# lich0031/AIDE

Hardware: AMD Instinct MI355X
Metric: training images/sec FuseUNet 256x256x2 bs=4/GPU (higher is better)
Workload: dtype f32; 1 GPU; c2 fuseunet fwd+loss+bwd+Adam(amsgrad), 256x256 2-modal, bs=4/GPU, fp32; global_batch=4, parallelism=dp1

## Files before the change

aide_amd/build.py:

```python
import hashlib
import os
import subprocess
import sys
from concurrent.futures import ThreadPoolExecutor

HERE = os.path.dirname(os.path.abspath(__file__))
CSRC = os.path.join(HERE, 'csrc')
OBJ = os.path.join(HERE, 'build')
LIB = os.path.join(HERE, 'libaide_hip.so')
SOURCES = ['conv3x3.hip', 'conv3x3_winograd.hip', 'conv3x3_wino4.hip', 'conv3x3_wgrad.hip', 'conv3x3_wgrad4.hip', 'conv3x3_wgrad_stem.hip', 'conv3x3_bf16.hip', 'bn.hip', 'spatial.hip', 'loss.hip', 'loss_mc.hip', 'coteach_ext.hip', 'head_adam.hip',
           'convt.hip', 'attention.hip', 'ktimer.hip', 'eval3d.hip', 'augment.hip', 'labelbank.hip', 'labelbank_image.hip', 'metrics_mc.hip']
FLAGS = ['--offload-arch=gfx950', '-O3', '-std=c++17', '-fPIC', '-ffp-contract=fast']


def _hipcc():
    for c in (os.environ.get('HIPCC'), '/opt/rocm/bin/hipcc', 'hipcc'):
        if c and (os.path.isabs(c) and os.path.exists(c) or not os.path.isabs(c)):
            return c
    raise RuntimeError('hipcc not found')


def _digest(paths):
    h = hashlib.sha1()
    for p in paths:
        with open(p, 'rb') as f:
            h.update(f.read())
    h.update(' '.join(FLAGS).encode())
    return h.hexdigest()


def build(force=False, verbose=True):
    os.makedirs(OBJ, exist_ok=True)
    hipcc = _hipcc()
    common = os.path.join(CSRC, 'common.h')

    def compile_one(src):
        sp = os.path.join(CSRC, src)
        op = os.path.join(OBJ, src.replace('.hip', '.o'))
        stamp = op + '.sha1'
        dg = _digest([sp, common])
        if not force and os.path.exists(op) and os.path.exists(stamp) and open(stamp).read() == dg:
            return op, False
        cmd = [hipcc] + FLAGS + ['-c', sp, '-o', op]
        r = subprocess.run(cmd, capture_output=True, text=True)
        if r.returncode != 0:
            raise RuntimeError('hipcc failed for %s:\n%s' % (src, r.stderr))
        with open(stamp, 'w') as f:
            f.write(dg)
        return op, True

    with ThreadPoolExecutor(max_workers=4) as ex:
        results = list(ex.map(compile_one, SOURCES))
    objs = [o for o, _ in results]
    if force or any(ch for _, ch in results) or not os.path.exists(LIB):
        r = subprocess.run([hipcc, '--offload-arch=gfx950', '-shared', '-fPIC', '-o', LIB] + objs,
                           capture_output=True, text=True)
        if r.returncode != 0:
            raise RuntimeError('link failed:\n' + r.stderr)
        if verbose:
            print('built', LIB)
    elif verbose:
        print('up to date', LIB)
    return LIB


if __name__ == '__main__':
    build(force='--force' in sys.argv)
```

aide_amd/csrc/conv3x3_wino4.hip:

```cpp
#include "common.h"
#include <stdlib.h>
#include <type_traits>

namespace {

template <int V> using ic = std::integral_constant<int, V>;

struct W4Args {
    const float* x;
    const float* u;
    const float* bias;
    float* y;
    long x_bs, y_bs, split_stride;
    int N, Cin, H, W, Cout;
    int blocks_w, blocks_h, n_co_tiles, splitk, stages_total, accumulate;
    int gp, gc;
    int pair;
    float* stats;
    const float* scale;
    int relu;
    const float* in_tab;
    int in_ng;
};

constexpr int F4_BNIN_MAXC = 1024;
constexpr int F4_NAGPR = 16;
constexpr int F4_RRS = 41;
constexpr int F4_RCS = 775;
constexpr int F4_RAW = 4 * F4_RCS;
constexpr int F4_V = 36 * 32 * 4;
constexpr int F4_SET = F4_RAW + F4_V;
constexpr int F4_LDS = 2 * F4_SET > 4 * 128 * 64 ? 2 * F4_SET : 4 * 128 * 64;

__host__ __device__ constexpr int f4_pos(int q, int b) {
    return 6 * (q / 3) + ((q % 3) == 0 ? 1 + b : (q % 3) == 1 ? 3 + b : 5 * b);
}
__host__ __device__ constexpr int f4_slot(int c) { return c == 0 ? 4 : c == 5 ? 5 : c - 1; }

__device__ __forceinline__ void bt6(float d0, float d1, float d2, float d3, float d4, float d5, float* o, int st) {
    const float a = __builtin_fmaf(-4.f, d2, d4), b = __builtin_fmaf(4.f, d1, -d3);
    const float c = d4 - d2, e = d3 - d1;
    o[0] = __builtin_fmaf(-5.f, d2, __builtin_fmaf(4.f, d0, d4));
    o[st] = a - b;
    o[2 * st] = a + b;
    o[3 * st] = __builtin_fmaf(2.f, e, c);
    o[4 * st] = __builtin_fmaf(-2.f, e, c);
    o[5 * st] = __builtin_fmaf(-5.f, d3, __builtin_fmaf(4.f, d1, d5));
}

template <int CTRL, int ROW_MASK>
__device__ __forceinline__ float dpp_add(float v) {
    return v + __builtin_bit_cast(float, __builtin_amdgcn_update_dpp(0, __builtin_bit_cast(int, v), CTRL, ROW_MASK, 0xf, true));
}
__device__ __forceinline__ float half_total_dpp(float v) {
    v = dpp_add<0x111, 0xf>(v);
    v = dpp_add<0x112, 0xf>(v);
    v = dpp_add<0x114, 0xf>(v);
    v = dpp_add<0x118, 0xf>(v);
    v = dpp_add<0x142, 0xa>(v);
    return v;
}

template <int MODE, bool AFF = false, bool BNIN = false>
__global__ __launch_bounds__(256, 1) void conv3x3_wino4_kernel(const W4Args a) {
    extern __shared__ __attribute__((aligned(16))) float lds[];
    const int tid = threadIdx.x, lane = tid & 63;
    const int wid = __builtin_amdgcn_readfirstlane(tid >> 6);
    const int half = lane >> 5, j = lane & 31;
    const int ph = wid & 1, cb = wid >> 1;

    int b = xcd_remap(blockIdx.x, gridDim.x);
    const int p_in = b % a.gp;            b /= a.gp;
    const int co_in = b % a.gc;           b /= a.gc;
    const int ncg = a.n_co_tiles / a.gc;
    const int cog = b % ncg;              b /= ncg;
    const int split = b % a.splitk;       b /= a.splitk;
    const int co_tile = cog * a.gc + co_in;
    int pt = b * a.gp + p_in;
    const int tw = pt % a.blocks_w;       pt /= a.blocks_w;
    const int th = pt % a.blocks_h;
    const int n = pt / a.blocks_h;
    constexpr int PAIR = MODE == 1;
    constexpr bool canv = MODE == 2;
    constexpr int NR = canv ? 22 : 18, NI = canv ? 5 : 8, RRS = canv ? 29 : F4_RRS;
    constexpr int TPH = canv ? 20 : 16, TPW = canv ? 20 : 32;
    static_assert(NR * RRS <= F4_RCS, "raw channel plane");
    const int h0 = th * TPH, w0 = tw * TPW, co0 = co_tile * 64;
    const int HW = a.H * a.W;
    constexpr int pair = PAIR;

    const int sps = a.stages_total / a.splitk;
    const int s_begin = split * sps;
    const int s_end = min(s_begin + sps, a.stages_total);

    constexpr int NUI = 4 * NR * NI, NUE = 4 * NR * 2;
    unsigned offB[3], ldsB[3], offC, ldsC;
    int tabB[3], tabC;
#pragma unroll
    for (int e = 0; e < 3; ++e) {
        int q = tid + e * 256;
        while (q >= NUI) q -= 256;
        const int c = q / (NR * NI), rem = q - c * (NR * NI), r = rem / NI, s4 = rem - r * NI;
        const int ih = h0 - 1 + r, iw = w0 + 4 * s4;
        const int imgB = pair && s4 >= 4;
        const bool ok = ih >= 0 && ih < a.H && (pair || iw < a.W);
        offB[e] = ok ? (unsigned)((long)imgB * a.x_bs + c * HW + r * a.W + 1 + 4 * (pair ? (s4 & 3) : s4)) * 4u : BUF_OOB;
        ldsB[e] = (unsigned)(c * F4_RCS + r * RRS + 4 + 4 * s4 + 2 * imgB);
        tabB[e] = F4_LDS + (ok ? 0 : 2 * a.Cin) + 2 * c;
    }
    {
        int q = tid;
        if (q >= NUE) q -= NUE;
        const int c = q / (NR * 2), rem = q - c * (NR * 2), r = rem >> 1, side = rem & 1;
        const int ih = h0 - 1 + r, iw = side ? w0 + TPW : w0 - 1;
        const bool ok = !pair && ih >= 0 && ih < a.H && iw >= 0 && iw < a.W;
        tabC = F4_LDS + (ok ? 0 : 2 * a.Cin) + 2 * c;
        offC = ok ? (unsigned)(c * HW + r * a.W + (side ? TPW + 1 : 0)) * 4u : BUF_OOB;
        ldsC = (unsigned)(c * F4_RCS + r * RRS + (pair ? (side ? 21 : 20) : (side ? 4 + TPW : 3)));
    }
    const __amdgpu_buffer_rsrc_t xrs =
        make_rsrc(a.x + (long)(pair ? 2 * n : n) * a.x_bs + (long)h0 * a.W + w0 - (a.W + 1));
    const long ubase = ((long)9 * ph * 2 * a.Cout + co0 + cb * 32) * 4;
    const __amdgpu_buffer_rsrc_t urs = __builtin_amdgcn_make_buffer_rsrc(
        const_cast<float*>(a.u + ubase), 0, (int)(((long)a.Cin * 36 * a.Cout - ubase) * 4), 0x00020000);
    const unsigned uoff = (unsigned)(half * a.Cout + j) * 16u;
    const unsigned upos = (unsigned)a.Cout * 32u;

    f32x4 rb[3];
    float rc;
    f32x4 ua[2][9];
    auto fetch_u = [&](int q, int stage, f32x4* dst) {
        const unsigned us = ((unsigned)min(stage, s_end - 1) * 18u + (unsigned)q) * upos;
        dst[q] = buf_load_f32x4(urs, uoff, us);
    };
    auto fetch = [&](int l, int stage) {
        const unsigned xs = (unsigned)(min(stage, s_end - 1) * 4) * (unsigned)HW * 4u;
        if (l < 3) rb[l] = buf_load_f32x4(xrs, offB[l], xs);
        else rc = buf_load_f32(xrs, offC, xs);
    };
    auto put_raw = [&](int w, float* raw) {
        if (w < 12) raw[ldsB[w >> 2] + (w & 3)] = rb[w >> 2][w & 3];
        else raw[ldsC] = rc;
    };
    f32x2 tv[4];
    auto bn_tab = [&](int stage) {
        const int so = min(stage, s_end - 1) * 8;
#pragma unroll
        for (int e = 0; e < 3; ++e) tv[e] = *reinterpret_cast<const f32x2*>(lds + tabB[e] + so);
        tv[3] = *reinterpret_cast<const f32x2*>(lds + tabC + so);
    };
    auto bn_in = [&]() {
#pragma unroll
        for (int e = 0; e < 3; ++e) {
            const f32x2 sc = f32x2{tv[e].x, tv[e].x}, sh = f32x2{tv[e].y, tv[e].y};
            const f32x2 lo = f32x2{rb[e].x, rb[e].y} * sc + sh, hi = f32x2{rb[e].z, rb[e].w} * sc + sh;
            rb[e] = f32x4{fmaxf(lo.x, 0.f), fmaxf(lo.y, 0.f), fmaxf(hi.x, 0.f), fmaxf(hi.y, 0.f)};
        }
        rc = fmaxf(__builtin_fmaf(rc, tv[3].x, tv[3].y), 0.f);
    };
    if constexpr (BNIN) {
        float* tab = lds + F4_LDS;
        const float* src = a.in_tab + (long)(n / a.in_ng) * 2 * a.Cin;
        for (int i = tid; i < 2 * a.Cin; i += 256) { tab[i] = src[i]; tab[2 * a.Cin + i] = 0.f; }
        __syncthreads();
    }

    const int item = tid & 127, hs = wid >> 1;
    const int tslot = canv ? min(item >> 2, 24) : (item >> 2);
    const int trow = canv ? tslot / 5 : tslot >> 3, tcol = canv ? tslot - 5 * trow : tslot & 7;
    const int xr_off = (item & 3) * F4_RCS + trow * 4 * RRS + 3 + 4 * tcol + ((pair && tcol >= 4) ? 2 : 0);
    f32x2 tp[6][3];
    f32x2 tq[9];
    auto xf_read = [&](int i, int xo) {
        const float v = lds[xo + (i / 6) * RRS + (i % 6)];
        if ((i % 6) & 1) tp[i / 6][(i % 6) >> 1].y = v; else tp[i / 6][(i % 6) >> 1].x = v;
    };
    auto xf_half = [&](auto HS) {
        constexpr int khs = decltype(HS)::value;
        f32x2 T[3][3];
#pragma unroll
        for (int cp = 0; cp < 3; ++cp) {
            const f32x2 d0 = tp[0][cp], d1 = tp[1][cp], d2 = tp[2][cp], d3 = tp[3][cp], d4 = tp[4][cp], d5 = tp[5][cp];
            if (khs == 0) {
                const f32x2 aa = d4 - 4.f * d2, bb = 4.f * d1 - d3;
                T[0][cp] = (4.f * d0 + d4) - 5.f * d2;
                T[1][cp] = bb * f32x2{-1.f, -1.f} + aa;
                T[2][cp] = aa + bb;
            } else {
                const f32x2 cc = d2 * f32x2{-1.f, -1.f} + d4, ee = d1 * f32x2{-1.f, -1.f} + d3;
// ... 78 lines not shown
            if constexpr (BNIN) {
                if (st == 24) bn_tab(s + 2);
                if (st == 30) bn_in();
            }
            if (st >= PR && st < PR + 5) {
#pragma unroll
                for (int q = 0; q < 3; ++q)
                    if (3 * (st - PR) + q < 13) put_raw(3 * (st - PR) + q, sc);
            }
            __builtin_amdgcn_sched_barrier(0);
        }
        __syncthreads();
    };
    for (int s = s_begin; s < s_end; s += 2) {
        stage(s, set0, set1, ic<0>{});
        stage(s + 1, set1, set0, ic<1>{});
    }

    float* xbuf = lds;
    float* yn = a.y + (long)split * a.split_stride + (long)(pair ? 2 * n + ((j & 7) >> 2) : n) * a.y_bs;
    const bool add_bias = (a.bias != nullptr) && (split == 0);
    const int oh = h0 + 4 * (canv ? j / 5 : j >> 3), ow = pair ? 4 * (j & 3) : w0 + 4 * (canv ? j % 5 : j & 7);
    const bool pok = (!canv || j < 25) && oh < a.H && ow < a.W;
    auto epilogue = [&](auto PH) {
        constexpr int kph = decltype(PH)::value;
        auto partial = [&](int r, f32x2* yp) {
            f32x2 T[3][4];
#pragma unroll
            for (int i = 0; i < 3; ++i) {
                auto m = [&](int c) { return f32x2{acc[6 * i + f4_slot(c)][r], acc[6 * i + f4_slot(c)][r + 1]}; };
                const f32x2 m0 = m(0), m1 = m(1), m2 = m(2), m3 = m(3), m4 = m(4), m5 = m(5);
                const f32x2 s12 = m1 + m2, d12 = m2 * f32x2{-1.f, -1.f} + m1, s34 = m3 + m4, d34 = m4 * f32x2{-1.f, -1.f} + m3;
                T[i][0] = m0 + s12 + s34;
                T[i][1] = d34 * f32x2{2.f, 2.f} + d12;
                T[i][2] = s34 * f32x2{4.f, 4.f} + s12;
                T[i][3] = d34 * f32x2{8.f, 8.f} + d12 + m5;
            }
#pragma unroll
            for (int bq = 0; bq < 4; ++bq) {
                if (kph == 0) {
                    const f32x2 sm = T[1][bq] + T[2][bq], df = T[2][bq] * f32x2{-1.f, -1.f} + T[1][bq];
                    yp[bq] = T[0][bq] + sm; yp[4 + bq] = df; yp[8 + bq] = sm; yp[12 + bq] = df;
                } else {
                    const f32x2 sm = T[0][bq] + T[1][bq], df = T[1][bq] * f32x2{-1.f, -1.f} + T[0][bq];
                    yp[bq] = sm; yp[4 + bq] = df * f32x2{2.f, 2.f}; yp[8 + bq] = sm * f32x2{4.f, 4.f};
                    yp[12 + bq] = df * f32x2{8.f, 8.f} + T[2][bq];
                }
            }
        };
        f32x2* const xbuf2 = reinterpret_cast<f32x2*>(xbuf);
#pragma unroll
        for (int rp = 0; rp < 4; ++rp) {
            f32x2 yp[16];
            partial(2 * rp + 8 * (1 - kph), yp);
#pragma unroll
            for (int o = 0; o < 16; ++o) xbuf2[((wid * 64) + rp * 16 + o) * 64 + lane] = yp[o];
        }
        __syncthreads();
        float bvs[8];
#pragma unroll
        for (int q = 0; q < 8; ++q) {
            const int r = q + 8 * kph;
            const int co = co0 + cb * 32 + (r & 3) + 8 * (r >> 2) + 4 * half;
            bvs[q] = (add_bias && co < a.Cout) ? a.bias[co] : 0.f;
        }
        float svs[8];
        if constexpr (AFF) {
#pragma unroll
            for (int q = 0; q < 8; ++q) {
                const int r = q + 8 * kph;
                const int co = co0 + cb * 32 + (r & 3) + 8 * (r >> 2) + 4 * half;
                svs[q] = co < a.Cout ? a.scale[co] : 1.f;
            }
        }
#pragma unroll
        for (int rp = 0; rp < 4; ++rp) {
            f32x2 yp[16];
            partial(2 * rp + 8 * kph, yp);
#pragma unroll
            for (int o = 0; o < 16; ++o) yp[o] += xbuf2[(((wid ^ 1) * 64) + rp * 16 + o) * 64 + lane];
#pragma unroll
            for (int e = 0; e < 2; ++e) {
                const int r = 2 * rp + e + 8 * kph;
                const int co = co0 + cb * 32 + (r & 3) + 8 * (r >> 2) + 4 * half;
                if (a.stats) {
                    float s1 = 0.f, s2 = 0.f;
                    if (pok) {
#pragma unroll
                        for (int o = 0; o < 16; ++o) { s1 += yp[o][e]; s2 = __builtin_fmaf(yp[o][e], yp[o][e], s2); }
                    }
                    s1 = half_total_dpp(s1);
                    s2 = half_total_dpp(s2);
                    if (j == 31 && co < a.Cout) {
                        const int nparts = a.N * a.blocks_h * a.blocks_w, blk = (n * a.blocks_h + th) * a.blocks_w + tw;
                        *reinterpret_cast<f32x2*>(a.stats + ((long)co * nparts + blk) * 2) = f32x2{s1, s2};
                    }
                }
                if (pok && co < a.Cout) {
                    const float bv = bvs[2 * rp + e];
                    f32x4* const p0 = reinterpret_cast<f32x4*>(yn + (long)co * HW + (long)oh * a.W + ow);
                    f32x4 o[4];
#pragma unroll
                    for (int i = 0; i < 4; ++i)
                        o[i] = f32x4{yp[4 * i][e] + bv, yp[4 * i + 1][e] + bv, yp[4 * i + 2][e] + bv, yp[4 * i + 3][e] + bv};
                    if constexpr (AFF) {
                        const float sv = svs[2 * rp + e];
#pragma unroll
                        for (int i = 0; i < 4; ++i) {
#pragma unroll
                            for (int k = 0; k < 4; ++k) {
                                const float v = __builtin_fmaf(yp[4 * i + k][e], sv, bv);
                                o[i][k] = a.relu ? fmaxf(v, 0.f) : v;
                            }
                        }
                    }
                    if (a.accumulate) {
                        f32x4 old[4];
#pragma unroll
                        for (int i = 0; i < 4; ++i) old[i] = *reinterpret_cast<const f32x4*>(reinterpret_cast<const float*>(p0) + (long)i * a.W);
#pragma unroll
                        for (int i = 0; i < 4; ++i) o[i] += old[i];
                    }
#pragma unroll
                    for (int i = 0; i < 4; ++i) *reinterpret_cast<f32x4*>(reinterpret_cast<float*>(p0) + (long)i * a.W) = o[i];
                }
            }
        }
    };
    if (ph == 0) epilogue(ic<0>{}); else epilogue(ic<1>{});
    };
    if (hs == 0) run(ic<0>{}); else run(ic<1>{});
}

__global__ __launch_bounds__(256) void w4_splitk_reduce_kernel(const float* __restrict__ slabs, long split_stride,
                                                               int splitk, float* __restrict__ y, long y_bs, int C,
                                                               int HW, const float* __restrict__ bias, int accumulate,
                                                               long total4, const float* __restrict__ scale, int relu) {
    for (long i = (long)blockIdx.x * 256 + threadIdx.x; i < total4; i += (long)gridDim.x * 256) {
        const long e = i * 4, chw = (long)C * HW;
        const long n = e / chw, rem = e - n * chw;
        f32x4 v = *reinterpret_cast<const f32x4*>(slabs + e);
        for (int s = 1; s < splitk; ++s) v += *reinterpret_cast<const f32x4*>(slabs + (long)s * split_stride + e);
        if (scale) {
            const float sv = scale[rem / HW], bv = bias[rem / HW];
#pragma unroll
            for (int k = 0; k < 4; ++k) { const float t = __builtin_fmaf(v[k], sv, bv); v[k] = relu ? fmaxf(t, 0.f) : t; }
        } else if (bias) { const float bv = bias[rem / HW]; v += f32x4{bv, bv, bv, bv}; }
        f32x4* p = reinterpret_cast<f32x4*>(y + n * y_bs + rem);
        if (accumulate) v += *p;
        *p = v;
    }
}

__device__ __forceinline__ void wino4_g(const float g[9], float u[36]) {
    float t[18];
#pragma unroll
    for (int c = 0; c < 3; ++c) {
        const float g0 = g[c], g1 = g[3 + c], g2 = g[6 + c];
        const float s = g0 + g2;
        t[c] = 0.25f * g0;
        t[3 + c] = (-1.f / 6.f) * (s + g1);
        t[6 + c] = (-1.f / 6.f) * (s - g1);
        const float q = __builtin_fmaf(4.f, g2, g0);
        t[9 + c] = (1.f / 24.f) * (q + 2.f * g1);
        t[12 + c] = (1.f / 24.f) * (q - 2.f * g1);
        t[15 + c] = g2;
    }
#pragma unroll
    for (int r = 0; r < 6; ++r) {
        const float a0 = t[r * 3], a1 = t[r * 3 + 1], a2 = t[r * 3 + 2];
        const float s = a0 + a2, q = __builtin_fmaf(4.f, a2, a0);
        u[r * 6] = 0.25f * a0;
        u[r * 6 + 1] = (-1.f / 6.f) * (s + a1);
        u[r * 6 + 2] = (-1.f / 6.f) * (s - a1);
        u[r * 6 + 3] = (1.f / 24.f) * (q + 2.f * a1);
        u[r * 6 + 4] = (1.f / 24.f) * (q - 2.f * a1);
        u[r * 6 + 5] = a2;
    }
}

struct W4PackDesc {
    const float* w; float* uf; float* ud;
    int Co, Ci, pad0, pad1;
    long block_start;
};

constexpr int P4_T = 32;
__global__ __launch_bounds__(128) void wino4_pack_multi_kernel(const W4PackDesc* __restrict__ descs, int n, long total_blocks) {
    __shared__ __attribute__((aligned(16))) float ot[36 * 128];
    for (long blk = blockIdx.x; blk < total_blocks; blk += gridDim.x) {
    int lo = 0, hi = n - 1;
    while (lo < hi) {
        const int mid = (lo + hi + 1) >> 1;
        if (descs[mid].block_start <= blk) lo = mid; else hi = mid - 1;
    }
    const W4PackDesc d = descs[lo];
    const int tid = threadIdx.x;
    const int tiles_ci = (d.Ci + P4_T - 1) / P4_T;
    const int tb = (int)(blk - d.block_start);
    const int co0 = (tb / tiles_ci) * P4_T, ci0 = (tb % tiles_ci) * P4_T;
    const int nci = min(P4_T, d.Ci - ci0);
    float g[9], u[36];
    const int lo2 = tid & 3, hi5 = tid >> 2;
    for (int grp = 0; grp < 16; ++grp) {
        const bool fwd = grp < 8;
        const int q = grp & 7;
        float* dst = fwd ? d.uf : d.ud;
        if (dst == nullptr) continue;
        const int co = fwd ? hi5 : 4 * q + lo2, ci = fwd ? 4 * q + lo2 : hi5;
        const bool live = fwd ? (ci0 + 4 * q < d.Ci) : (co0 + 4 * q < d.Co);
        if (!live) continue;
        {
            const bool in = co0 + co < d.Co && ci < nci;
            const float* wp = d.w + ((long)(co0 + co) * d.Ci + ci0 + ci) * 9;
#pragma unroll
            for (int t = 0; t < 9; ++t) g[t] = in ? wp[fwd ? t : 8 - t] : 0.f;
        }
        wino4_g(g, u);
        const int otid = (lo2 >> 1) * 64 + hi5 * 2 + (lo2 & 1);
#pragma unroll
        for (int p = 0; p < 36; ++p) ot[p * 128 + otid] = u[p];
        __syncthreads();
        const int C = fwd ? d.Co : d.Ci, c0 = fwd ? co0 : ci0;
        const long gbase = (long)((fwd ? ci0 : co0) / 4 + q) * 18;
        const int nrow = min(P4_T, C - c0);
#pragma unroll
        for (int k = 0; k < 9; ++k) {
            const int f = tid + k * 128, pq = f >> 6, hh = (f >> 5) & 1, row = f & 31;
            if (row < nrow) {
                const float* o0 = ot + f4_pos(pq, 0) * 128 + hh * 64 + row * 2;
                const float* o1 = ot + f4_pos(pq, 1) * 128 + hh * 64 + row * 2;
                *reinterpret_cast<f32x4*>(dst + (((gbase + pq) * 2 + hh) * C + c0 + row) * 4) =
                    f32x4{o0[0], o0[1], o1[0], o1[1]};
            }
        }
        __syncthreads();
    }
    }
}

}

extern "C" {

int aide_conv3x3_wino4_supported(int Cin, int H, int W, int Cout) {
    return (H % 4 == 0 && W % 4 == 0 && H >= 16 && W >= 16 && Cout % 32 == 0 &&
            Cin % 8 == 0) ? 1 : 0;
}

static int f4_mode(int H, int W, int* bh, int* bw) {
    const int sh = (H + 15) / 16, sw = (W + 31) / 32, ch = (H + 19) / 20, cw = (W + 19) / 20;
    const int mode = W == 16 ? 1 : ((long)ch * cw < (long)sh * sw) ? 2 : 0;
    *bh = mode == 2 ? ch : sh;
    *bw = mode == 2 ? cw : sw;
    return mode;
}

int aide_conv3x3_wino4_splitk(int N, int Cin, int H, int W, int Cout) {
    int bh, bw;
    f4_mode(H, W, &bh, &bw);
    const long nb = (long)bh * bw * (W == 16 ? N / 2 : N) * ((Cout + 63) / 64);
    const int pairs = Cin / 8;
    const long target = 200;
    int s = 1;
    while (nb * s < target && pairs % (s * 2) == 0 && s * 2 <= pairs / 4) s *= 2;
    return s;
}

int aide_conv3x3_wino4_stats_parts(int N, int H, int W) {
    int bh, bw;
    f4_mode(H, W, &bh, &bw);
    return W < 32 ? 0 : N * bh * bw;
}

int aide_conv3x3_wino4_pack_blocks(int Co, int Ci) {
    return ((Co + P4_T - 1) / P4_T) * ((Ci + P4_T - 1) / P4_T);
}

int aide_conv3x3_wino4_pack_multi(const void* descs, int n, int64_t total_blocks, hipStream_t stream) {
    if (!descs || n <= 0 || total_blocks <= 0) return AIDE_ERR_ARG;
    static_assert(sizeof(W4PackDesc) == 48, "descriptor layout");
    const long grid = total_blocks;
    AIDE_LAUNCH_TIMED(AIDE_KT_OTHER, 0.0, wino4_pack_multi_kernel, dim3((unsigned)grid), dim3(128), 0, stream,
                       (const W4PackDesc*)descs, n, (long)total_blocks);
    return aide_launch_status();
}

int aide_conv3x3_wino4(const float* x, int64_t x_bs, const float* u, const float* bias, float* y,
                       int64_t y_bs, int N, int Cin, int H, int W, int Cout, int accumulate, int splitk,
                       float* ws, float* stats_parts, const float* epi_scale, int epi_relu, const float* in_bn_tab,
                       int in_bn_group_images, hipStream_t stream) {
    const float* aff = epi_scale;
    const int aff_relu = aff ? epi_relu : 0;
    if (!x || !u || !y || !aide_conv3x3_wino4_supported(Cin, H, W, Cout) || x_bs % 4 || y_bs % 4 || (W == 16 && N % 2))
        return AIDE_ERR_ARG;
    static AideLdsOptIn lds_opt;
    if (int rc = lds_opt.ensure([] {
            constexpr int plain = F4_LDS * (int)sizeof(float), bnin = (F4_LDS + 4 * F4_BNIN_MAXC) * (int)sizeof(float);
            const struct { const void* fn; int bytes; } ks[] = {
                {(const void*)conv3x3_wino4_kernel<0>, plain}, {(const void*)conv3x3_wino4_kernel<1>, plain},
                {(const void*)conv3x3_wino4_kernel<2>, plain}, {(const void*)conv3x3_wino4_kernel<0, true>, plain},
                {(const void*)conv3x3_wino4_kernel<2, true>, plain}, {(const void*)conv3x3_wino4_kernel<0, false, true>, bnin},
                {(const void*)conv3x3_wino4_kernel<2, false, true>, bnin}};
            for (const auto& k : ks) {
                const hipError_t e = hipFuncSetAttribute(k.fn, hipFuncAttributeMaxDynamicSharedMemorySize, k.bytes);
                if (e != hipSuccess) return e;
            }
            return hipSuccess;
        })) return rc;
    W4Args a;
    if (stats_parts && !(splitk <= 1 && accumulate == 0 && W >= 32)) return AIDE_ERR_ARG;
    a.stats = stats_parts;
    const int mode = f4_mode(H, W, &a.blocks_h, &a.blocks_w);
    if (aff && (accumulate != 0 || !bias || (mode == 1 && splitk <= 1))) return AIDE_ERR_ARG;
    a.scale = splitk > 1 ? nullptr : aff;
    a.relu = aff_relu;
    a.pair = mode == 1 ? 1 : 0;
    if (in_bn_tab && (mode == 1 || aff || Cin > F4_BNIN_MAXC || in_bn_group_images < 1 || N % in_bn_group_images)) return AIDE_ERR_ARG;
    a.in_tab = in_bn_tab; a.in_ng = in_bn_tab ? in_bn_group_images : 1;
    a.x = x; a.u = u; a.x_bs = x_bs; a.N = N; a.Cin = Cin; a.H = H; a.W = W; a.Cout = Cout;
    a.n_co_tiles = (Cout + 63) / 64;
    a.stages_total = Cin / 4;
    if (splitk < 1) splitk = 1;
    if ((Cin / 8) % splitk != 0) return AIDE_ERR_ARG;
    if (splitk > 1 && !ws) return AIDE_ERR_ARG;
    a.splitk = splitk;
    if (splitk > 1) {
        a.y = ws; a.y_bs = (long)Cout * H * W; a.split_stride = (long)N * Cout * H * W;
        a.bias = nullptr; a.accumulate = 0;
    } else {
        a.y = y; a.y_bs = y_bs; a.split_stride = 0; a.bias = bias; a.accumulate = (accumulate == 1);
    }
    const long nb = (long)a.blocks_w * a.blocks_h * (a.pair ? N / 2 : N) * a.n_co_tiles * splitk;
    {
        const long P = (long)a.blocks_w * a.blocks_h * (a.pair ? N / 2 : N);
        const int C = a.n_co_tiles;
        const long per_xcd = nb / 8 > 0 ? nb / 8 : 1;
        const double ub = 144.0 * (double)Cin * Cout, xb = 1.44 * 4.0 * (double)N * Cin * H * W;
        long bp = 1; int bc = C;
        double best = 1e300;
        const bool grouped = AIDE_CONV_FLOPS(N, H, W, Cout, Cin) >= 8e9;
        for (long gp = 1; gp <= P && gp <= per_xcd && grouped; gp *= 2) {
            if (P % gp) continue;
            for (int gc = 1; gc <= C; ++gc) {
                if (C % gc || gp * gc > per_xcd) continue;
                const double cost = ub * (double)P / (double)gp + xb * (double)C / (double)gc;
                if (cost < best) { best = cost; bp = gp; bc = gc; }
            }
        }
        a.gp = (int)bp; a.gc = bc;
    }
    if (a.in_tab) {
        const size_t lds_bytes = (F4_LDS + 4 * (size_t)Cin) * sizeof(float);
        if (mode == 2) {
            AIDE_LAUNCH_TIMED(AIDE_KT_WINO4, AIDE_CONV_FLOPS(N, H, W, Cout, Cin), (conv3x3_wino4_kernel<2, false, true>),
                              dim3((unsigned)nb), dim3(256), lds_bytes, stream, a);
        } else {
            AIDE_LAUNCH_TIMED(AIDE_KT_WINO4, AIDE_CONV_FLOPS(N, H, W, Cout, Cin), (conv3x3_wino4_kernel<0, false, true>),
                              dim3((unsigned)nb), dim3(256), lds_bytes, stream, a);
        }
    } else if (a.scale && mode == 2) {
        AIDE_LAUNCH_TIMED(AIDE_KT_WINO4, AIDE_CONV_FLOPS(N, H, W, Cout, Cin), (conv3x3_wino4_kernel<2, true>), dim3((unsigned)nb),
                          dim3(256), F4_LDS * sizeof(float), stream, a);
    } else if (a.scale) {
        AIDE_LAUNCH_TIMED(AIDE_KT_WINO4, AIDE_CONV_FLOPS(N, H, W, Cout, Cin), (conv3x3_wino4_kernel<0, true>), dim3((unsigned)nb),
                          dim3(256), F4_LDS * sizeof(float), stream, a);
    } else if (a.pair) {
        AIDE_LAUNCH_TIMED(AIDE_KT_WINO4, AIDE_CONV_FLOPS(N, H, W, Cout, Cin), conv3x3_wino4_kernel<1>, dim3((unsigned)nb), dim3(256),
                          F4_LDS * sizeof(float), stream, a);
    } else if (mode == 2) {
        AIDE_LAUNCH_TIMED(AIDE_KT_WINO4, AIDE_CONV_FLOPS(N, H, W, Cout, Cin), conv3x3_wino4_kernel<2>, dim3((unsigned)nb), dim3(256),
                          F4_LDS * sizeof(float), stream, a);
    } else {
        AIDE_LAUNCH_TIMED(AIDE_KT_WINO4, AIDE_CONV_FLOPS(N, H, W, Cout, Cin), conv3x3_wino4_kernel<0>, dim3((unsigned)nb), dim3(256),
                          F4_LDS * sizeof(float), stream, a);
    }
    int rc = aide_launch_status();
    if (rc != 0) return rc;
    if (splitk > 1 && accumulate != 2) {
        const long total4 = (long)N * Cout * H * W / 4;
        AIDE_LAUNCH_TIMED(AIDE_KT_REDUCE, 0.0, w4_splitk_reduce_kernel, dim3((unsigned)min((total4 + 255) / 256, 4096L)), dim3(256), 0,
                           stream, ws, (long)N * Cout * H * W, splitk, y, (long)y_bs, Cout, H * W, bias, accumulate,
                           total4, aff, aff_relu);
        rc = aide_launch_status();
    }
    return rc;
}

}
```

aide_amd/csrc/conv3x3_winograd.hip:

```cpp
#include "common.h"

namespace {

struct WinoArgs {
    const float* x;
    const float* u;
    const float* bias;
    float* y;
    long x_bs, y_bs, split_stride;
    int N, Cin, H, W, Cout;
    int tiles_w, tiles_h, n_co_tiles, splitk, chunks_total, accumulate;
};

constexpr int WCK = 8;
constexpr int WTCO = 64;
constexpr int RROWS = 18, RRS = 24;
constexpr int RCS = RROWS * RRS + 8;
constexpr int RAWL = WCK * RCS;
constexpr int VL = 16 * 64 * WCK;
constexpr int UL = 16 * WTCO * WCK;
constexpr int WBUF = RAWL + VL + UL;

__global__ __launch_bounds__(256, 1) void conv3x3_wino_kernel(const WinoArgs a) {
    extern __shared__ __attribute__((aligned(16))) float lds[];
    const int tid = threadIdx.x, lane = tid & 63, wid = tid >> 6;
    const int half = lane >> 5, j = lane & 31;
    const int wave_m = wid >> 1, wave_n = wid & 1;

    int b = xcd_remap(blockIdx.x, gridDim.x);
    const int co_tile = b % a.n_co_tiles; b /= a.n_co_tiles;
    const int split = b % a.splitk;       b /= a.splitk;
    const int tw = b % a.tiles_w;         b /= a.tiles_w;
    const int th = b % a.tiles_h;
    const int n = b / a.tiles_h;
    const int h0 = th * 16, w0 = tw * 16, co0 = co_tile * WTCO;
    const int HW = a.H * a.W;

    const int cps = (a.chunks_total + a.splitk - 1) / a.splitk;
    const int c_begin = split * cps;
    const int c_end = min(c_begin + cps, a.chunks_total);

    constexpr int NRB = 3, NRC = 2, NU = UL / 4 / 256;
    unsigned offB[NRB], ldsB[NRB], offC[NRC], ldsC[NRC], offU[NU];
#pragma unroll
    for (int e = 0; e < NRB; ++e) {
        int q = tid + e * 256;
        if (q >= WCK * RROWS * 4) q -= 256;
        const int c = q / (RROWS * 4), rem = q - c * (RROWS * 4), r = rem / 4, s4 = rem - r * 4;
        const int ih = h0 - 1 + r, iw = w0 + 4 * s4;
        const bool ok = ih >= 0 && ih < a.H && iw < a.W;
        offB[e] = ok ? (unsigned)(c * HW + r * a.W + 1 + 4 * s4) * 4u : BUF_OOB;
        ldsB[e] = (unsigned)(c * RCS + r * RRS + 4 + 4 * s4);
    }
#pragma unroll
    for (int e = 0; e < NRC; ++e) {
        int q = tid + e * 256;
        if (q >= WCK * RROWS * 2) q -= 256;
        const int c = q / (RROWS * 2), rem = q - c * (RROWS * 2), r = rem / 2, side = rem - r * 2;
        const int ih = h0 - 1 + r, iw = side ? w0 + 16 : w0 - 1;
        const bool ok = ih >= 0 && ih < a.H && iw >= 0 && iw < a.W;
        offC[e] = ok ? (unsigned)(c * HW + r * a.W + (side ? 17 : 0)) * 4u : BUF_OOB;
        ldsC[e] = (unsigned)(c * RCS + r * RRS + (side ? 20 : 3));
    }
#pragma unroll
    for (int v = 0; v < NU; ++v) {
        const int f = tid + v * 256;
        const int pp = f / (WTCO * WCK / 4), w4 = f - pp * (WTCO * WCK / 4);
        offU[v] = (unsigned)(pp * a.Cout * WCK + w4 * 4) * 4u;
    }
    const __amdgpu_buffer_rsrc_t xrs =
        make_rsrc(a.x + (long)n * a.x_bs + (long)h0 * a.W + w0 - (a.W + 1));
    const __amdgpu_buffer_rsrc_t urs = make_rsrc(a.u + (long)co0 * WCK);

    f32x4 rb[NRB], ru[NU];
    float rc[NRC];
    auto fetch_raw = [&](int l, int chunk) {
        const unsigned xs = (unsigned)(min(chunk, c_end - 1) * WCK) * (unsigned)HW * 4u;
        if (l < NRB) rb[l] = buf_load_f32x4(xrs, offB[l], xs);
        else rc[l - NRB] = buf_load_f32(xrs, offC[l - NRB], xs);
    };
    auto put_raw = [&](int l, float* raw) {
        if (l < NRB) *reinterpret_cast<f32x4*>(raw + ldsB[l]) = rb[l];
        else raw[ldsC[l - NRB]] = rc[l - NRB];
    };
    auto fetch_u = [&](int v, int chunk) {
        const unsigned us = (unsigned)min(chunk, c_end - 1) * 16u * (unsigned)a.Cout * (unsigned)WCK * 4u;
        ru[v] = buf_load_f32x4(urs, offU[v], us);
    };
    auto put_u = [&](int v, float* ubuf) { *reinterpret_cast<f32x4*>(ubuf + (tid + v * 256) * 4) = ru[v]; };

    f32x2 td[16], to[16];
    const int xci = lane & 7, xtj = lane >> 3;
    const int xr_off = xci * RCS + 4 * wid * RRS + 3 + 2 * xtj;
    const int xw_off = (2 * wid * 8 + xtj) * WCK + xci;
    auto xf_read = [&](int i, const float* raw) {
        td[i].x = raw[xr_off + (i / 4) * RRS + (i % 4)];
        td[i].y = raw[xr_off + (2 + i / 4) * RRS + (i % 4)];
    };
    auto xf_math = [&]() {
        f32x2 tt[16];
#pragma unroll
        for (int c = 0; c < 4; ++c) {
            tt[c] = td[c] - td[8 + c]; tt[4 + c] = td[4 + c] + td[8 + c];
            tt[8 + c] = td[8 + c] - td[4 + c]; tt[12 + c] = td[4 + c] - td[12 + c];
        }
#pragma unroll
        for (int r = 0; r < 4; ++r) {
            to[r * 4] = tt[r * 4] - tt[r * 4 + 2]; to[r * 4 + 1] = tt[r * 4 + 1] + tt[r * 4 + 2];
            to[r * 4 + 2] = tt[r * 4 + 2] - tt[r * 4 + 1]; to[r * 4 + 3] = tt[r * 4 + 1] - tt[r * 4 + 3];
        }
    };
    auto xf_store = [&](int o, float* vbuf) {
        vbuf[o * 64 * WCK + xw_off] = to[o].x;
        vbuf[o * 64 * WCK + xw_off + 8 * WCK] = to[o].y;
    };

    f32x16 acc[16];
#pragma unroll
    for (int p = 0; p < 16; ++p)
#pragma unroll
        for (int r = 0; r < 16; ++r) acc[p][r] = 0.0f;

    float* set0 = lds;
    float* set1 = lds + WBUF;
#pragma unroll
    for (int l = 0; l < NRB + NRC; ++l) fetch_raw(l, c_begin);
#pragma unroll
    for (int v = 0; v < NU; ++v) fetch_u(v, c_begin);
#pragma unroll
    for (int l = 0; l < NRB + NRC; ++l) put_raw(l, set0);
#pragma unroll
    for (int v = 0; v < NU; ++v) put_u(v, set0 + RAWL + VL);
#pragma unroll
    for (int l = 0; l < NRB + NRC; ++l) fetch_raw(l, c_begin + 1);
    __syncthreads();
#pragma unroll
    for (int i = 0; i < 16; ++i) xf_read(i, set0);
    xf_math();
#pragma unroll
    for (int o = 0; o < 16; ++o) xf_store(o, set0 + RAWL);
#pragma unroll
    for (int l = 0; l < NRB + NRC; ++l) put_raw(l, set1);
    __syncthreads();

    int cur = 0;
    for (int chunk = c_begin; chunk < c_end; ++chunk) {
        float* sc = cur ? set1 : set0;
        float* sn = cur ? set0 : set1;
        const float* la = sc + RAWL + VL + (wave_m * 32 + j) * WCK + half * 4;
        const float* lb = sc + RAWL + (wave_n * 32 + j) * WCK + half * 4;
        constexpr int STEPS = 16 * (WCK / 2);
        f32x4 a0A, b0A, a1A, b1A, a0B, b0B, a1B, b1B;
        auto frag = [&](int p, f32x4& af, f32x4& bf) {
            af = *reinterpret_cast<const f32x4*>(la + p * WTCO * WCK);
            bf = *reinterpret_cast<const f32x4*>(lb + p * 64 * WCK);
        };
        auto slot = [&](int st, const f32x4& a0c, const f32x4& b0c, const f32x4& a1c, const f32x4& b1c,
                        f32x4& a0n, f32x4& b0n, f32x4& a1n, f32x4& b1n) {
            const int g2 = st >> 3, k = st & 7, q = k >> 1;
            if (k == 0 && g2 + 1 < 8) { frag(2 * g2 + 2, a0n, b0n); frag(2 * g2 + 3, a1n, b1n); }
            if (k & 1) acc[2 * g2 + 1] = __builtin_amdgcn_mfma_f32_32x32x2f32(a1c[q], b1c[q], acc[2 * g2 + 1], 0, 0, 0);
            else acc[2 * g2] = __builtin_amdgcn_mfma_f32_32x32x2f32(a0c[q], b0c[q], acc[2 * g2], 0, 0, 0);
            if (st < NU) fetch_u(st, chunk + 1);
            else if (st < NU + NRB + NRC) fetch_raw(st - NU, chunk + 2);
            if (st >= 4 && st < 20) xf_read(st - 4, sn);
            if (st == 24) xf_math();
            if (st >= 26 && st < 42) xf_store(st - 26, sn + RAWL);
            if (st >= 44 && st < 44 + NU) put_u(st - 44, sn + RAWL + VL);
            if (st >= 52 && st < 52 + NRB + NRC) put_raw(st - 52, sc);
            __builtin_amdgcn_sched_barrier(0);
        };
        frag(0, a0A, b0A); frag(1, a1A, b1A);
#pragma unroll
        for (int st = 0; st < STEPS; st += 16) {
#pragma unroll
            for (int k = 0; k < 8; ++k) slot(st + k, a0A, b0A, a1A, b1A, a0B, b0B, a1B, b1B);
#pragma unroll
            for (int k = 0; k < 8; ++k) slot(st + 8 + k, a0B, b0B, a1B, b1B, a0A, b0A, a1A, b1A);
        }
        __syncthreads();
        cur ^= 1;
    }

    float* yn = a.y + (long)split * a.split_stride + (long)n * a.y_bs;
    const bool add_bias = (a.bias != nullptr) && (split == 0);
    const int tile = wave_n * 32 + j, ti = tile >> 3, tj = tile & 7;
    const int oh = h0 + 2 * ti, ow = w0 + 2 * tj;
    const bool pok = oh < a.H && ow < a.W;
    float bvs[16];
#pragma unroll
    for (int r = 0; r < 16; ++r) {
        const int co = co0 + wave_m * 32 + (r & 3) + 8 * (r >> 2) + 4 * half;
        bvs[r] = (add_bias && pok && co < a.Cout) ? a.bias[co] : 0.f;
    }
#pragma unroll
    for (int r4 = 0; r4 < 16; r4 += 4) {
        float2 olds[4][2];
#pragma unroll
        for (int q = 0; q < 4; ++q) {
            const int co = co0 + wave_m * 32 + q + 8 * (r4 >> 2) + 4 * half;
#pragma unroll
            for (int i = 0; i < 2; ++i)
                olds[q][i] = (a.accumulate && pok && co < a.Cout)
                                 ? *reinterpret_cast<const float2*>(yn + (long)co * HW + (long)(oh + i) * a.W + ow) : make_float2(0.f, 0.f);
        }
#pragma unroll
        for (int q = 0; q < 4; ++q) {
            const int r = r4 + q;
            const int co = co0 + wave_m * 32 + (r & 3) + 8 * (r >> 2) + 4 * half;
            float s[2][4];
#pragma unroll
            for (int c = 0; c < 4; ++c) {
                const float m0 = acc[c][r], m1 = acc[4 + c][r], m2 = acc[8 + c][r], m3 = acc[12 + c][r];
                s[0][c] = m0 + m1 + m2;
                s[1][c] = m1 - m2 - m3;
            }
            if (pok && co < a.Cout) {
                const float bv = bvs[r];
#pragma unroll
                for (int i = 0; i < 2; ++i) {
                    float2 o;
                    o.x = s[i][0] + s[i][1] + s[i][2] + bv;
                    o.y = s[i][1] - s[i][2] - s[i][3] + bv;
                    float2* p = reinterpret_cast<float2*>(yn + (long)co * HW + (long)(oh + i) * a.W + ow);
                    o.x += olds[q][i].x; o.y += olds[q][i].y;
                    *p = o;
                }
            }
        }
    }
}

__global__ void wino_splitk_reduce_kernel(const float* __restrict__ slabs, long split_stride, int splitk,
                                          float* __restrict__ y, long y_bs, int C, int HW,
                                          const float* __restrict__ bias, int accumulate, long total) {
    for (long i = (long)blockIdx.x * blockDim.x + threadIdx.x; i < total;
         i += (long)gridDim.x * blockDim.x) {
        const long chw = (long)C * HW;
        const long n = i / chw, rem = i - n * chw;
        float v = slabs[i];
        for (int s = 1; s < splitk; ++s) v += slabs[(long)s * split_stride + i];
        if (bias) v += bias[rem / HW];
        float* p = y + n * y_bs + rem;
        if (accumulate) v += *p;
        *p = v;
    }
}
__global__ __launch_bounds__(256) void wino_splitk_reduce4_kernel(const float* __restrict__ slabs, long split_stride, int splitk,
                                                                  float* __restrict__ y, long y_bs, int C, int HW,
                                                                  const float* __restrict__ bias, int accumulate, long total4) {
    const long i = (long)blockIdx.x * blockDim.x + threadIdx.x;
    if (i >= total4) return;
    const long chw4 = (long)C * HW / 4;
    const long n = i / chw4, rem = (i - n * chw4) * 4;
    const float* sp = slabs + i * 4;
    f32x4 v = *reinterpret_cast<const f32x4*>(sp);
    int s = 1;
    for (; s + 4 <= splitk; s += 4) {
        const f32x4 t0 = *reinterpret_cast<const f32x4*>(sp + (long)s * split_stride);
        const f32x4 t1 = *reinterpret_cast<const f32x4*>(sp + (long)(s + 1) * split_stride);
        const f32x4 t2 = *reinterpret_cast<const f32x4*>(sp + (long)(s + 2) * split_stride);
        const f32x4 t3 = *reinterpret_cast<const f32x4*>(sp + (long)(s + 3) * split_stride);
        v = (((v + t0) + t1) + t2) + t3;
    }
    for (; s < splitk; ++s) v += *reinterpret_cast<const f32x4*>(sp + (long)s * split_stride);
    if (bias) v += bias[rem / HW];
    float* p = y + n * y_bs + rem;
    if (accumulate) v += *reinterpret_cast<const f32x4*>(p);
    *reinterpret_cast<f32x4*>(p) = v;
}

struct WinoPackDesc {
    const float* w; float* uf; float* ud;
    int Co, Ci, ci_pad, co_pad;
    long block_start;
};

__device__ __forceinline__ void wino_g(const float g[9], float u[16]) {
    float t[12];
#pragma unroll
    for (int c = 0; c < 3; ++c) {
        const float g0 = g[c], g1 = g[3 + c], g2 = g[6 + c];
        t[c] = g0; t[3 + c] = 0.5f * (g0 + g1 + g2); t[6 + c] = 0.5f * (g0 - g1 + g2); t[9 + c] = g2;
    }
#pragma unroll
    for (int r = 0; r < 4; ++r) {
        const float a0 = t[r * 3], a1 = t[r * 3 + 1], a2 = t[r * 3 + 2];
        u[r * 4] = a0; u[r * 4 + 1] = 0.5f * (a0 + a1 + a2); u[r * 4 + 2] = 0.5f * (a0 - a1 + a2); u[r * 4 + 3] = a2;
    }
}

constexpr int WP_T = 32;
__global__ __launch_bounds__(256) void wino_pack_multi_kernel(const WinoPackDesc* __restrict__ descs, int n) {
    __shared__ __attribute__((aligned(16))) float ot[16 * 256];
    const long blk = blockIdx.x;
    int lo = 0, hi = n - 1;
    while (lo < hi) {
        const int mid = (lo + hi + 1) >> 1;
        if (descs[mid].block_start <= blk) lo = mid; else hi = mid - 1;
    }
    const WinoPackDesc d = descs[lo];
    const int tid = threadIdx.x;
    const int tiles_ci = (d.Ci + WP_T - 1) / WP_T;
    const int tb = (int)(blk - d.block_start);
    const int co0 = (tb / tiles_ci) * WP_T, ci0 = (tb % tiles_ci) * WP_T;
    const int nci = min(WP_T, d.Ci - ci0);
    float g[9], u[16];
    const int lo3 = tid & 7, hi5 = tid >> 3;
    for (int grp = 0; grp < 8; ++grp) {
        const bool fwd = grp < 4;
        const int q = grp & 3;
        float* dst = fwd ? d.uf : d.ud;
        if (dst == nullptr) continue;
        const int co = fwd ? hi5 : 8 * q + lo3, ci = fwd ? 8 * q + lo3 : hi5;
        const bool live = fwd ? (ci0 + 8 * q < d.ci_pad) : (co0 + 8 * q < d.co_pad);
        if (!live) continue;
        {
            const bool in = co0 + co < d.Co && ci < nci;
            const float* wp = d.w + ((long)(co0 + co) * d.Ci + ci0 + ci) * 9;
#pragma unroll
            for (int t = 0; t < 9; ++t) g[t] = in ? wp[fwd ? t : 8 - t] : 0.f;
        }
        wino_g(g, u);
#pragma unroll
        for (int p = 0; p < 16; ++p) ot[p * 256 + tid] = u[p];
        __syncthreads();
        const int C = fwd ? d.Co : d.Ci, c0 = fwd ? co0 : ci0;
        const long gbase = (long)((fwd ? ci0 : co0) / 8 + q) * 16;
        const int nrun = min(WP_T, C - c0) * 8;
#pragma unroll
        for (int k = 0; k < 4; ++k) {
            const int f = tid + k * 256, p = f >> 6, x4 = (f & 63) * 4;
            if (x4 < nrun)
                *reinterpret_cast<f32x4*>(dst + ((gbase + p) * C + c0) * 8 + x4) =
                    *reinterpret_cast<const f32x4*>(ot + p * 256 + x4);
        }
        __syncthreads();
    }
}

}

extern "C" {

int aide_conv3x3_wino_supported(int Cin, int H, int W, int Cout) {
    return (H % 2 == 0 && W % 4 == 0 && Cout % 64 == 0 && Cin % 8 == 0) ? 1 : 0;
}

int aide_conv3x3_wino_splitk(int N, int Cin, int H, int W, int Cout) {
    const long nb = (long)((H + 15) / 16) * ((W + 15) / 16) * N * (Cout / 64);
    const int chunks = Cin / 8;
    int s = 1;
    while (nb * s < 200 && s * 2 <= chunks / 4) s *= 2;
    return s;
}

int aide_conv3x3_wino_pack_blocks(int Co, int Ci) {
    return ((Co + WP_T - 1) / WP_T) * ((Ci + WP_T - 1) / WP_T);
}

int aide_conv3x3_wino_pack_multi(const void* descs, int n, int64_t total_blocks, hipStream_t stream) {
    if (!descs || n <= 0 || total_blocks <= 0) return AIDE_ERR_ARG;
    static_assert(sizeof(WinoPackDesc) == 48, "descriptor layout");
    AIDE_LAUNCH_TIMED(AIDE_KT_OTHER, 0.0, wino_pack_multi_kernel, dim3((unsigned)total_blocks), dim3(256), 0, stream,
                       (const WinoPackDesc*)descs, n);
    return aide_launch_status();
}

int aide_conv3x3_wino(const float* x, int64_t x_bs, const float* u, const float* bias, float* y,
                      int64_t y_bs, int N, int Cin, int H, int W, int Cout, int accumulate, int splitk,
                      float* ws, hipStream_t stream) {
    if (!x || !u || !y || !aide_conv3x3_wino_supported(Cin, H, W, Cout) || x_bs % 4 || y_bs % 2)
        return AIDE_ERR_ARG;
    static AideLdsOptIn lds_opt;
    if (int rc = lds_opt.ensure([] {
            return hipFuncSetAttribute((const void*)conv3x3_wino_kernel, hipFuncAttributeMaxDynamicSharedMemorySize,
                                       2 * WBUF * (int)sizeof(float));
        })) return rc;
    WinoArgs a;
    a.x = x; a.u = u; a.x_bs = x_bs; a.N = N; a.Cin = Cin; a.H = H; a.W = W; a.Cout = Cout;
    a.tiles_w = (W + 15) / 16; a.tiles_h = (H + 15) / 16; a.n_co_tiles = Cout / WTCO;
    a.chunks_total = Cin / WCK;
    if (splitk < 1) splitk = 1;
    if (splitk > a.chunks_total) splitk = a.chunks_total;
    if (splitk > 1 && !ws) return AIDE_ERR_ARG;
    a.splitk = splitk;
    if (splitk > 1) {
        a.y = ws; a.y_bs = (long)Cout * H * W; a.split_stride = (long)N * Cout * H * W;
        a.bias = nullptr; a.accumulate = 0;
    } else {
        a.y = y; a.y_bs = y_bs; a.split_stride = 0; a.bias = bias; a.accumulate = (accumulate == 1);
    }
    const long nb = (long)a.tiles_w * a.tiles_h * N * a.n_co_tiles * splitk;
    AIDE_LAUNCH_TIMED(AIDE_KT_WINO2, AIDE_CONV_FLOPS(N, H, W, Cout, Cin), conv3x3_wino_kernel, dim3((unsigned)nb), dim3(256),
                      2 * WBUF * sizeof(float), stream, a);
    int rc = aide_launch_status();
    if (rc != 0) return rc;
    if (splitk > 1 && accumulate != 2) {
        const long total = (long)N * Cout * H * W;
        if ((H * W) % 4 == 0 && y_bs % 4 == 0) {
            AIDE_LAUNCH_TIMED(AIDE_KT_REDUCE, 0.0, wino_splitk_reduce4_kernel, dim3((unsigned)((total / 4 + 255) / 256)), dim3(256), 0, stream, ws,
                               total, splitk, y, (long)y_bs, Cout, H * W, bias, accumulate, total / 4);
        } else {
            const int blocks = (int)min((total + 255) / 256, (long)2048);
            AIDE_LAUNCH_TIMED(AIDE_KT_REDUCE, 0.0, wino_splitk_reduce_kernel, dim3(blocks), dim3(256), 0, stream, ws,
                               total, splitk, y, (long)y_bs, Cout, H * W, bias, accumulate, total);
        }
        rc = aide_launch_status();
    }
    return rc;
}

}
```

aide_amd/csrc/head_adam.hip:

```cpp
#include "common.h"

namespace {

constexpr int MAXK = 8;
constexpr int HEAD_WG_BLOCKS = 1024;

template <int K, typename XT>
__global__ __launch_bounds__(256) void head_fwd_kernel(const XT* __restrict__ x, long x_bs,
                                                       const float* __restrict__ w, const float* __restrict__ b,
                                                       float* __restrict__ y, long y_bs, int C, int HW,
                                                       long total4, const float* __restrict__ in_scale,
                                                       const float* __restrict__ in_shift) {
    extern __shared__ float ws[];
    for (int i = threadIdx.x; i < K * C; i += 256) ws[i] = w[i];
    __syncthreads();
    const int hw4 = HW / 4;
    for (long i = (long)blockIdx.x * 256 + threadIdx.x; i < total4; i += (long)gridDim.x * 256) {
        const long n = i / hw4, p = i - n * hw4;
        const XT* xp = x + n * x_bs + p * 4;
        f32x4 acc[K];
#pragma unroll
        for (int k = 0; k < K; ++k) { const float bk = b ? b[k] : 0.f; acc[k] = f32x4{bk, bk, bk, bk}; }
        for (int c = 0; c < C; ++c) {
            f32x4 v = ld4(xp + (long)c * HW);
            if (in_scale) {
                const float sc = in_scale[c], sh = in_shift[c];
#pragma unroll
                for (int e = 0; e < 4; ++e) v[e] = fmaxf(__builtin_fmaf(v[e], sc, sh), 0.0f);
            }
#pragma unroll
            for (int k = 0; k < K; ++k) acc[k] += ws[k * C + c] * v;
        }
#pragma unroll
        for (int k = 0; k < K; ++k) *reinterpret_cast<f32x4*>(y + n * y_bs + (long)k * HW + p * 4) = acc[k];
    }
}

template <int K, typename DT>
__global__ __launch_bounds__(256) void head_dgrad_kernel(const float* __restrict__ dy, long dy_bs,
                                                         const float* __restrict__ w, DT* __restrict__ dx,
                                                         long dx_bs, int C, int HW, long total4) {
    extern __shared__ float ws[];
    for (int i = threadIdx.x; i < K * C; i += 256) ws[i] = w[i];
    __syncthreads();
    const int hw4 = HW / 4;
    for (long i = (long)blockIdx.x * 256 + threadIdx.x; i < total4; i += (long)gridDim.x * 256) {
        const long n = i / hw4, p = i - n * hw4;
        f32x4 g[K];
#pragma unroll
        for (int k = 0; k < K; ++k) g[k] = *reinterpret_cast<const f32x4*>(dy + n * dy_bs + (long)k * HW + p * 4);
        DT* xp = dx + n * dx_bs + p * 4;
        for (int c = 0; c < C; ++c) {
            f32x4 v = ws[c] * g[0];
#pragma unroll
            for (int k = 1; k < K; ++k) {
                const float wk = ws[k * C + c];
                v = f32x4{__builtin_fmaf(wk, g[k][0], v[0]), __builtin_fmaf(wk, g[k][1], v[1]), __builtin_fmaf(wk, g[k][2], v[2]),
                          __builtin_fmaf(wk, g[k][3], v[3])};
            }
            st4(xp + (long)c * HW, v);
        }
    }
}

template <int K, typename XT>
__global__ __launch_bounds__(256) void head_wgrad_kernel(const float* __restrict__ dy, long dy_bs,
                                                         const XT* __restrict__ x, long x_bs, int C, int HW,
                                                         long total4, double* __restrict__ partials,
                                                         const float* __restrict__ in_scale, const float* __restrict__ in_shift) {
    constexpr int G = K > 4 ? 4 : 8;
    __shared__ double sm[4][G * K];
    const int hw4 = HW / 4;
    const int lane = threadIdx.x & 63, wid = threadIdx.x >> 6;
    const int stride = gridDim.x * 256;
    for (int c0 = -1; c0 < C; c0 += G) {
        double acc[G][K];
#pragma unroll
        for (int g = 0; g < G; ++g)
#pragma unroll
            for (int k = 0; k < K; ++k) acc[g][k] = 0.0;
        for (long i = (long)blockIdx.x * 256 + threadIdx.x; i < total4; i += stride) {
            const long n = i / hw4, p = i - n * hw4;
            f32x4 gk[K];
#pragma unroll
            for (int k = 0; k < K; ++k) gk[k] = *reinterpret_cast<const f32x4*>(dy + n * dy_bs + (long)k * HW + p * 4);
            f32x4 v[G];
#pragma unroll
            for (int g = 0; g < G; ++g) {
                const int c = c0 + g;
                v[g] = f32x4{1.f, 1.f, 1.f, 1.f};
                if (c >= 0 && c < C) {
                    v[g] = ld4(x + n * x_bs + (long)c * HW + p * 4);
                    if (in_scale) {
                        const float sc = in_scale[c], sh = in_shift[c];
#pragma unroll
                        for (int e = 0; e < 4; ++e) v[g][e] = fmaxf(__builtin_fmaf(v[g][e], sc, sh), 0.0f);
                    }
                }
            }
#pragma unroll
            for (int g = 0; g < G; ++g)
#pragma unroll
                for (int k = 0; k < K; ++k)
                    acc[g][k] += (double)(gk[k][0] * v[g][0] + gk[k][1] * v[g][1] + (gk[k][2] * v[g][2] + gk[k][3] * v[g][3]));
        }
#pragma unroll
        for (int g = 0; g < G; ++g)
#pragma unroll
            for (int k = 0; k < K; ++k) acc[g][k] = wave_sum_d(acc[g][k]);
        __syncthreads();
        if (lane == 0)
#pragma unroll
            for (int g = 0; g < G; ++g)
#pragma unroll
                for (int k = 0; k < K; ++k) sm[wid][g * K + k] = acc[g][k];
        __syncthreads();
        if (threadIdx.x < G * K) {
            const int g = threadIdx.x / K, k = threadIdx.x - g * K, c = c0 + g;
            if (c < C) {
                const double t = sm[0][threadIdx.x] + sm[1][threadIdx.x] + sm[2][threadIdx.x] + sm[3][threadIdx.x];
                const int slot = (c >= 0) ? k * C + c : K * C + k;
                partials[(long)blockIdx.x * (K * C + K) + slot] = t;
            }
        }
    }
}

__global__ __launch_bounds__(64) void head_wgrad_finalize_kernel(const double* __restrict__ partials, int nblocks,
                                                                 int KC, int K, float* __restrict__ dw,
                                                                 float* __restrict__ db) {
    const int i = blockIdx.x;
    double s = 0.0;
    for (int b = threadIdx.x; b < nblocks; b += 64) s += partials[(long)b * (KC + K) + i];
    s = wave_sum_d(s);
    if (threadIdx.x == 0) {
        if (i < KC) dw[i] = (float)s;
        else if (db) db[i - KC] = (float)s;
    }
}

struct AdamArgs {
    float* const* p; const float* const* g; float* const* m; float* const* v; float* const* vmax;
    const long* sizes; const long* block_start;
    int ntensors;
    float lr, beta1, beta2, eps, weight_decay, bc1, bc2_sqrt;
    int amsgrad;
};

__global__ __launch_bounds__(256) void adam_kernel(const AdamArgs a) {
    const long blk = blockIdx.x;
    int lo = 0, hi = a.ntensors - 1;
    while (lo < hi) {
        const int mid = (lo + hi + 1) >> 1;
        if (a.block_start[mid] <= blk) lo = mid; else hi = mid - 1;
    }
    const int t = lo;
    const long base = (blk - a.block_start[t]) * 1024;
    const long n = a.sizes[t];
    float* p = a.p[t]; const float* g = a.g[t];
    float* m = a.m[t]; float* v = a.v[t]; float* vm = a.vmax[t];
#pragma unroll
    for (int k = 0; k < 4; ++k) {
        const long i = base + k * 256 + threadIdx.x;
        if (i < n) {
            float gi = g[i];
            const float pi = p[i];
            if (a.weight_decay != 0.f) gi += a.weight_decay * pi;
            const float mi = a.beta1 * m[i] + (1.f - a.beta1) * gi;
            const float vi = a.beta2 * v[i] + (1.f - a.beta2) * gi * gi;
            m[i] = mi; v[i] = vi;
            float vhat = vi;
            if (a.amsgrad) { vhat = fmaxf(vm[i], vi); vm[i] = vhat; }
            const float denom = sqrtf(vhat) / a.bc2_sqrt + a.eps;
            p[i] = pi - (a.lr / a.bc1) * (mi / denom);
        }
    }
}

int grid_for(long total) { return (int)max(1L, min((total + 255) / 256, 4096L)); }

template <int K, typename XT>
int head_wgrad_launch(const float* dy, long dy_bs, const XT* x, long x_bs, int C, int HW, long total4,
                      double* partials, int nblocks, hipStream_t s, const float* in_scale = nullptr, const float* in_shift = nullptr) {
    AIDE_LAUNCH_TIMED(AIDE_KT_OTHER, 0.0, (head_wgrad_kernel<K, XT>), dim3(nblocks), dim3(256), 0, s, dy, dy_bs, x, x_bs, C, HW,
                       total4, partials, in_scale, in_shift);
    return aide_launch_status();
}

template <typename XT>
int head_fwd_t(const XT* x, int64_t x_bs, const float* w, const float* b, float* y, int64_t y_bs, int N, int C, int K,
               int H, int W, hipStream_t stream, const float* in_scale = nullptr, const float* in_shift = nullptr) {
    const int HW = H * W;
    if (K < 1 || K > MAXK || HW % 4 || x_bs % 4 || y_bs % 4) return AIDE_ERR_ARG;
    const long total4 = (long)N * HW / 4;
    const int grid = grid_for(total4);
    const size_t sh = (size_t)K * C * sizeof(float);
    aide_pick<1, 2, 3, 4, 5, 6, 7, 8>(K, [&](auto k) {
        AIDE_LAUNCH_TIMED(AIDE_KT_OTHER, 0.0, (head_fwd_kernel<k(), XT>), dim3(grid), dim3(256), sh, stream, x, (long)x_bs, w, b, y,
                          (long)y_bs, C, HW, total4, in_scale, in_shift);
    });
    return aide_launch_status();
}

template <typename XT, typename DT>
int head_bwd_t(const float* dy, int64_t dy_bs, const XT* x, int64_t x_bs, const float* w, DT* dx, int64_t dx_bs,
               float* dw, float* db, int N, int C, int K, int H, int W, void* ws, hipStream_t stream,
               const float* in_scale = nullptr, const float* in_shift = nullptr) {
    const int HW = H * W;
    if (K < 1 || K > MAXK || HW % 4 || x_bs % 4 || dy_bs % 4 || (dx && dx_bs % 4) || !ws) return AIDE_ERR_ARG;
    const long total4 = (long)N * HW / 4;
    const size_t sh = (size_t)K * C * sizeof(float);
    if (dx) {
        const int grid = grid_for(total4);
        aide_pick<1, 2, 3, 4, 5, 6, 7, 8>(K, [&](auto k) {
            AIDE_LAUNCH_TIMED(AIDE_KT_OTHER, 0.0, (head_dgrad_kernel<k(), DT>), dim3(grid), dim3(256), sh, stream, dy, (long)dy_bs, w, dx,
                              (long)dx_bs, C, HW, total4);
        });
    }
    if (!dw) return aide_launch_status();
    const int nblocks = (int)max(1L, min((total4 + 255) / 256, (long)HEAD_WG_BLOCKS));
    const int rc = aide_pick<1, 2, 3, 4, 5, 6, 7, 8>(K, [&](auto k) {
        return head_wgrad_launch<k()>(dy, dy_bs, x, x_bs, C, HW, total4, (double*)ws, nblocks, stream, in_scale, in_shift);
    });
    if (rc) return rc;
    AIDE_LAUNCH_TIMED(AIDE_KT_OTHER, 0.0, head_wgrad_finalize_kernel, dim3(K * C + K), dim3(64), 0, stream,
                       (const double*)ws, nblocks, K * C, K, dw, db);
    return aide_launch_status();
}

}

extern "C" {

size_t aide_head1x1_ws_bytes(int C, int K) { return (size_t)HEAD_WG_BLOCKS * (K * C + K) * sizeof(double); }

int aide_head1x1_fwd_mixed(const void* x, int x_bf16, int64_t x_bs, const float* w, const float* b, float* y,
                           int64_t y_bs, int N, int C, int K, int H, int W, hipStream_t stream) {
    return aide_with_storage<bf16_store_t>(x_bf16, [&](auto xt) { return head_fwd_t(xt.cast(x), x_bs, w, b, y, y_bs, N, C, K, H, W, stream); });
}
int aide_head1x1_bwd_mixed(const float* dy, int64_t dy_bs, const void* x, int x_bf16, int64_t x_bs, const float* w,
                           void* dx, int dx_bf16, int64_t dx_bs, float* dw, float* db, int N, int C, int K, int H, int W,
                           void* ws, hipStream_t stream) {
    return aide_with_storage<bf16_store_t>(x_bf16, [&](auto xt) { return aide_with_storage<bf16_store_t>(dx_bf16, [&](auto dt) {
        return head_bwd_t(dy, dy_bs, xt.cast(x), x_bs, w, dt.cast(dx), dx_bs, dw, db, N, C, K, H, W, ws, stream);
    }); });
}

int aide_head1x1_fwd_bn(const float* z, int64_t z_bs, const float* in_scale, const float* in_shift, const float* w, const float* b,
                        float* y, int64_t y_bs, int N, int C, int K, int H, int W, hipStream_t stream) {
    if (!z || !in_scale || !in_shift) return AIDE_ERR_ARG;
    return head_fwd_t(z, z_bs, w, b, y, y_bs, N, C, K, H, W, stream, in_scale, in_shift);
}
int aide_head1x1_wgrad_bn(const float* dy, int64_t dy_bs, const float* z, int64_t z_bs, const float* in_scale, const float* in_shift,
                          float* dw, float* db, int N, int C, int K, int H, int W, void* ws, hipStream_t stream) {
    if (!z || !in_scale || !in_shift || !dw) return AIDE_ERR_ARG;
    return head_bwd_t<float, float>(dy, dy_bs, z, z_bs, nullptr, nullptr, 0, dw, db, N, C, K, H, W, ws, stream, in_scale, in_shift);
}

int aide_adam_amsgrad_multi(float* const* p, const float* const* g, float* const* m, float* const* v,
                            float* const* vmax, const int64_t* sizes, const int64_t* block_start,
                            int ntensors, int64_t total_blocks, float lr, float beta1, float beta2, float eps,
                            float weight_decay, int amsgrad, int64_t step, hipStream_t stream) {
    if (ntensors <= 0 || total_blocks <= 0 || step < 1) return AIDE_ERR_ARG;
    AdamArgs a;
    a.p = p; a.g = g; a.m = m; a.v = v; a.vmax = vmax;
    a.sizes = (const long*)sizes; a.block_start = (const long*)block_start; a.ntensors = ntensors;
    a.lr = lr; a.beta1 = beta1; a.beta2 = beta2; a.eps = eps; a.weight_decay = weight_decay;
    a.bc1 = (float)(1.0 - pow((double)beta1, (double)step));
    a.bc2_sqrt = (float)sqrt(1.0 - pow((double)beta2, (double)step));
    a.amsgrad = amsgrad;
    AIDE_LAUNCH_TIMED(AIDE_KT_OTHER, 0.0, adam_kernel, dim3((unsigned)total_blocks), dim3(256), 0, stream, a);
    return aide_launch_status();
}

}
```

aide_amd/engine.py:

```python
import ctypes

import torch

from . import ops
from ._lib import lib, check as _check
from .tape import Tape

PARAM_EPOCH = [0]
STATS_EPOCH = [0]


class GTensor(object):

    def __init__(self, name, channels, level, root=None, c0=0, is_input=False):
        self.name, self.C, self.level = name, channels, level
        self.root = root if root is not None else self
        self.c0 = c0
        self.is_input = is_input

    def slice(self, c0, channels, name=None):
        assert 0 <= c0 and c0 + channels <= self.C
        return GTensor(name or '%s[%d:%d]' % (self.name, c0, c0 + channels), channels, self.level,
                       self.root, self.c0 + c0)


class Graph(object):
    def __init__(self):
        self.roots, self.inputs, self.ops = [], [], []
        self.output = None

    def tensor(self, name, channels, level):
        t = GTensor(name, channels, level)
        self.roots.append(t)
        return t

    def input(self, name, channels):
        t = GTensor(name, channels, 0, is_input=True)
        self.inputs.append(t)
        return t

    def conv_bn_relu(self, src, dst, conv, bn, lane=0):
        self.ops.append(dict(kind='conv', src=src, dst=dst, conv=conv, bn=bn, lane=lane))

    def convT_bn_relu(self, src, dst, conv, bn):
        self.ops.append(dict(kind='convT', src=src, dst=dst, conv=conv, bn=bn))

    def pool(self, src, dst, lane_split=None):
        self.ops.append(dict(kind='pool', src=src, dst=dst, lane_split=lane_split))

    def upsample(self, src, dst):
        self.ops.append(dict(kind='up', src=src, dst=dst))

    def head(self, src, conv):
        self.ops.append(dict(kind='head', src=src, conv=conv))

    def spatial_attention(self, src, dst, mod):
        self.ops.append(dict(kind='sa', src=src, dst=dst, mod=mod))


FAMILIES = ops.FAMILIES
BF16 = ops.BF16
PACK_ORDER = (BF16, 4, 0, 2)
PRECISIONS = ('fp32', 'bf16')
import os as _os


class EngineConfig(object):
    DEFAULTS = dict(
        use_winograd=True,
        use_winograd_dgrad=True,
        use_winograd4=True,
        store_bf16=True,
        store_a_bf16=True,
        store_g_bf16=True,
        replay=_os.environ.get('AIDE_REPLAY', '1') != '0',
        shared_packs=True,
        fold_eval_bn=True,
        tail_wgrad_main=True,
        dual_fwd=True,
        free_lane=True,
        handover_on_kernel=True,
        w4_half_tile=True,
        grouped_bn=True,
        lazy_bn=True,
        direct_grads=_os.environ.get('AIDE_DIRECT_GRADS', '1') != '0',
        fuse_pool_bwd=True,
        fuse_head_bwd=True,
        lazy_head=True,
        fuse_pool_fwd=True,
    )

    def __init__(self, on_change=None):
        object.__setattr__(self, '_on_change', on_change)
        for k, v in self.DEFAULTS.items():
            object.__setattr__(self, k, v)

    def __setattr__(self, k, v):
        if k not in self.DEFAULTS:
            raise AttributeError('aide_amd: the engine has no switch %r (switches: %s)' % (k, ', '.join(sorted(self.DEFAULTS))))
        v = bool(v)
        if getattr(self, k) != v:
            object.__setattr__(self, k, v)
            if self._on_change is not None:
                self._on_change()

    def snapshot(self):
        return tuple(getattr(self, k) for k in sorted(self.DEFAULTS))


FLUSH_EVERY = 4


def conv_mode(cfg, n, cin, h, w, cout):
    if cfg.use_winograd and cfg.use_winograd4 and lib.aide_conv3x3_wino4_supported(cin, h, w, cout) and w != 16:
        flops = 2.0 * n * h * w * cin * cout * 9
        if cout % 64:
            return 0
        if flops >= 8e9 or cin * cout >= 128 * 128:
            return 4
    return 2 if use_winograd(cfg, n, cin, h, w, cout) else 0


WGRAD_OVERRIDE = {}


def use_winograd(cfg, n, cin, h, w, cout):
    return bool(cfg.use_winograd and lib.aide_conv3x3_wino_supported(cin, h, w, cout))


def select_conv(cfg, precision, training, groups, n, cin, cout, h, w, need_dgrad, stem_only_so_far):
    bf16 = precision == 'bf16'
    d = dict(wg_target=0, stats_parts=0)
    d['wino_f'] = conv_mode(cfg, n, cin, h, w, cout)
    d['wino_d'] = conv_mode(cfg, n, cout, h, w, cin) if (need_dgrad and cfg.use_winograd_dgrad) else 0
    if bf16 and FAMILIES[BF16].supported(cin, h, w, cout):
        d['wino_f'] = BF16
    if bf16 and need_dgrad and FAMILIES[BF16].supported(cout, h, w, cin):
        d['wino_d'] = BF16
    d['plan_f'] = FAMILIES[d['wino_f']].plan(n, cin, h, w, cout)
    d['plan_d'] = FAMILIES[d['wino_d']].plan(n, cout, h, w, cin) if need_dgrad else 0
    d['sk_f'] = lib.aide_conv3x3_ws_bytes(n, h, w, cout, d['plan_f'] >> 8)
    d['sk_d'] = lib.aide_conv3x3_ws_bytes(n, h, w, cin, d['plan_d'] >> 8) if need_dgrad else 0
    if bf16 and FAMILIES[BF16].wgrad_supported(cout, cin, h, w):
        d['wino_w'] = BF16
    elif cfg.use_winograd and cfg.use_winograd4 and (cout % 64 == 0 or cfg.w4_half_tile) and \
            WGRAD_OVERRIDE.get((cout, cin, h, w), 4) == 4 and FAMILIES[4].wgrad_supported(cout, cin, h, w):
        d['wino_w'] = 4
        if stem_only_so_far:
            d['wg_target'] = 256
    elif cfg.use_winograd and FAMILIES[2].wgrad_supported(cout, cin, h, w):
        d['wino_w'] = 2
    else:
        d['wino_w'] = 0
    d['wg_bytes'] = FAMILIES[d['wino_w']].wgrad_ws_bytes(n, cout, cin, h, w, **_wgrad_extra(d))
    if training and (d['plan_f'] >> 8) <= 1 \
            and (h * w) % 4 == 0 and lib.aide_bn_two_pass(n // max(groups, 1), cout, h, w):
        parts = lib.aide_conv3x3_wino4_stats_parts(n, h, w) if d['wino_f'] == 4 else 0
        d['stats_parts'] = max(parts, 0)
    d['fold'] = not training and cfg.fold_eval_bn and (
        (d['wino_f'] == 4 and w != 16) or (d['wino_f'] == 0 and (d['plan_f'] >> 8) <= 1))
    d['dz_bf16'] = (d['wino_w'] == BF16 and (not need_dgrad or d['wino_d'] == BF16) and cfg.store_bf16)
    d['z_bf16'] = d['wino_f'] == BF16 and cfg.store_bf16
    return d


def _wgrad_extra(st):
    return dict(target_wgs=256) if st.get('wg_target') else {}


def _pack_slot(mode, direction):
    return ('u' if mode else 'w') + direction


def _preferred(dev):
    from . import streams as _streams
    d = torch.device(dev)
    idx = d.index if d.index is not None else torch.cuda.current_device()
    pref = _streams.PREFERRED.get(idx)
    if pref is None:
        pref = _streams.PREFERRED[idx] = dict(side=torch.cuda.Stream(device=d), lane=torch.cuda.Stream(device=d))
    return pref


def _side_stream(dev):
    return _preferred(dev)['side']


class _Cover(object):

    def __init__(self):
        self.iv = []

    def write(self, c0, c1):
        covered = [(max(a, c0), min(b, c1)) for a, b in self.iv if a < c1 and b > c0]
        if not covered:
            self._add(c0, c1)
            return False, []
        gaps, cur = [], c0
        for a, b in sorted(covered):
            if a > cur:
                gaps.append((cur, a))
            cur = max(cur, b)
        if cur < c1:
            gaps.append((cur, c1))
        self._add(c0, c1)
        return True, gaps

    def _add(self, c0, c1):
        iv = sorted(self.iv + [(c0, c1)])
        out = [iv[0]]
        for a, b in iv[1:]:
            if a <= out[-1][1]:
                out[-1] = (out[-1][0], max(out[-1][1], b))
            else:
                out.append((a, b))
        self.iv = out


class Plan(object):
    def __init__(self, graph, params, n, h, w, device, training, precision='fp32', groups=1, shared=None, cfg=None):
        self.g, self.N, self.H, self.W, self.dev, self.training = graph, n, h, w, device, training
        cfg = self.cfg = cfg if cfg is not None else EngineConfig()
        self.precision = precision
        self._shared = shared if shared is not None else dict(buf={}, fresh={}, streams=None)
        self.groups = groups
        assert n % groups == 0
        bf16 = precision == 'bf16'
        self.pindex = {id(p): i for i, p in enumerate(params)}
        f32 = dict(device=device, dtype=torch.float32)
        forward_only = (groups > 1 or not training) and cfg.shared_packs

        def pack_buf(conv, direction, mode, make):
            key = (id(conv), direction, mode, device.index)
            t = self._shared['buf'].get(key)
            if t is None:
                t = self._shared['buf'][key] = make()
            return t
        self.act = {}
        self.grad = {}
        self.steps = []
        max_dz = max_wg = max_bnc = max_sk = 0
        stem_only = True
        for op in graph.ops:
            st = dict(op)
            if op['kind'] in ('conv', 'convT'):
                conv, src, dst = op['conv'], op['src'], op['dst']
                hh, ww = h >> dst.level, w >> dst.level
                cout = dst.C
                st['z'] = torch.empty(n, cout, hh, ww, **f32)
                for k in ('mean', 'rstd', 'scale', 'shift', 'fbias'):
                    st[k] = torch.empty(cout, **f32)
                max_dz = max(max_dz, n * cout * hh * ww)
                max_bnc = max(max_bnc, cout)
                if op['kind'] == 'conv':
                    cin = src.C
                    need_dg = not src.root.is_input and not forward_only
                    sel = select_conv(cfg, precision, training, groups, n, cin, cout, hh, ww, need_dg, stem_only)
                    max_sk = max(max_sk, sel.pop('sk_f'), sel.pop('sk_d'))
                    st.update(sel)
                    st['wf'] = st['wd'] = st['uf'] = st['ud'] = None
                    for direction, ci, co in [('f', cin, cout)] + ([('d', cout, cin)] if need_dg else []):
                        fam = FAMILIES[st['wino_' + direction]]
                        st[_pack_slot(fam.mode, direction)] = pack_buf(conv, direction, fam.mode,
                                                                       lambda: fam.pack_alloc(ci, co, device))
                    max_wg = max(max_wg, st['wg_bytes'])
                    st['stats'] = torch.empty(cout * st['stats_parts'] * 2, **f32) if st['stats_parts'] else None
                    st['pack_key'] = None
                    st['flops'] = 2.0 * n * hh * ww * cout * cin * 9
                    if st['z_bf16']:
                        st['z'] = torch.empty(n, cout, hh, ww, device=device, dtype=torch.bfloat16)
                else:
                    cin = src.C
                    st['wg_bytes'] = lib.aide_convT2x2_wgrad_ws_bytes(n, cin, cout, h >> src.level, w >> src.level)
                    max_wg = max(max_wg, st['wg_bytes'])
            elif op['kind'] == 'head':
                src = op['src']
                k = op['conv'].out_channels
                max_wg = max(max_wg, lib.aide_head1x1_ws_bytes(src.C, k))
            elif op['kind'] == 'sa':
                src, mod = op['src'], op['mod']
                hh, ww = h >> src.level, w >> src.level
                r = mod.conv1.out_channels
                for k in ('t1', 't2', 't3'):
                    st[k] = torch.empty(n, r, hh, ww, **f32)
                st['t4'] = torch.empty(n, 1, hh, ww, **f32)
                st['gate'] = torch.empty(n, hh, ww, **f32)
                st['stat'] = torch.empty(2, **f32)
            stem_only = stem_only and op['kind'] == 'conv' and op['src'].root.is_input
            self.steps.append(st)
        self._plan_lazy_bn()
        self._plan_lazy_head()
        narrow = {id(t): bf16 and cfg.store_a_bf16 for t in graph.roots}
        for st in self.steps:
            kind = st['kind']
            if kind == 'conv':
                if not (st['wino_f'] == BF16 and st['wino_w'] == BF16):
                    narrow[id(st['src'].root)] = False
            elif kind in ('convT', 'sa'):
                narrow[id(st['src'].root)] = False
            if kind == 'sa':
                narrow[id(st['dst'].root)] = False
        for t in graph.roots:
            dt = torch.bfloat16 if narrow.get(id(t)) else torch.float32
            self.act[id(t)] = torch.empty(n, t.C, h >> t.level, w >> t.level, device=device, dtype=dt)
        self._plan_pool_fwd()
        self.narrow_grad = {k: v and cfg.store_g_bf16 for k, v in narrow.items()}
        for st in self.steps:
            if st['kind'] == 'conv' and not st['src'].root.is_input and st['wino_d'] != BF16:
                self.narrow_grad[id(st['src'].root)] = False
        self.bn_ws = ops.bn_ws(max(max_bnc, 1), device)
        self.sk_ws = torch.empty(max(max_sk // 4, 1), **f32)
        self.lane_b = None
        if any(st.get('lane') for st in self.steps):
            pref = _preferred(device)
            self.lane_b = pref['lane'] if (pref is not None and pref.get('lane') is not None) else torch.cuda.Stream(device=device)
            self.bn_ws_b = ops.bn_ws(max(max_bnc, 1), device)
            self.sk_ws_b = torch.empty(max(max_sk // 4, 1), **f32)
            self.ev_lane_fork, self.ev_lane_join = ops.new_event(), ops.new_event()
            for st in self.steps:
                if st['kind'] == 'pool' and st.get('lane_split'):
                    st['ev_b'] = ops.new_event()
        self._max_dz, self._max_wg = max_dz, max_wg
        self.wg_ws = self.wg_queue = self._wq_active = None
        self._bwd_ready = False
        self.profiler = None
        self._pack_key, self._pack_tabs, self._pack_ids, self.side_fwd = None, {}, None, None
        self.side = _side_stream(device) if (training and groups == 1) else None
        self._convs = self._conv_wslots = None
        self._gate_conv = None
        self._tape_f = self._tape_b = None
        self._coef_key, self._coef_tensors, self._coef_ok, self._coef_next, self._coef_bns = None, None, False, None, []
        self._fp = None
        self._fp_slots = self._fp_bns = None
        self.overlap = True
        self.trace = None
        self.serial = 0
        self.key = None

    def _plan_lazy_bn(self):
        self.lazy_bn = 0
        if not (self.training and self.groups > 1) or not self.cfg.lazy_bn:
            return
        for st in self.steps:
            if st['kind'] != 'conv' or st.get('stats') is None:
                continue
            dst = st['dst']
            readers = [o for o in self.steps if o.get('src') is not None and o['src'].root is dst.root
                       and o['src'].c0 < dst.c0 + dst.C and dst.c0 < o['src'].c0 + o['src'].C]
            if len(readers) != 1:
                continue
            rd = readers[0]
            src = rd['src']
            if rd['kind'] != 'conv' or rd['wino_f'] != 4 or src.C > 1024 or not (src.c0 <= dst.c0 and dst.c0 + dst.C <= src.c0 + src.C):
                continue
            if rd.get('in_tab') is None:
                tab = torch.zeros(self.groups, src.C, 2, device=self.dev, dtype=torch.float32)
                tab[:, :, 0] = 1.0
                rd['in_tab'] = tab
            st['lazy_to'], st['tab_c0'] = rd, dst.c0 - src.c0
            st['z'] = None
            self.lazy_bn += 1

    def _plan_lazy_head(self):
        if not (self.training and self.groups == 1 and self.cfg.lazy_head and self.cfg.fuse_head_bwd):
            return
        for hst in self.steps:
            if hst['kind'] != 'head':
                continue
            src = hst['src']
            readers = [o for o in self.steps if o.get('src') is not None and o['src'].root is src.root
                       and o['src'].c0 < src.c0 + src.C and src.c0 < o['src'].c0 + o['src'].C]
            prods = [o for o in self.steps if o['kind'] == 'conv' and o['dst'].root is src.root
                     and (o['dst'].c0, o['dst'].C) == (src.c0, src.C)]
            if len(readers) != 1 or len(prods) != 1:
                continue
            o = prods[0]
            zn, zc, zh, zw = o['z'].shape
            if o.get('stats') is None or o['z'].dtype != torch.float32 or o.get('dz_bf16') or o.get('lazy_to') is not None or \
                    not lib.aide_bn_one_pass(zn, zc, zh, zw):
                continue
            o['head_lazy'] = True
            o['head_tab'] = torch.zeros(1, zc, 2, device=self.dev, dtype=torch.float32)
            hst['lazy_prod'] = o

    def _plan_pool_fwd(self):
        if not (self.training and self.cfg.fuse_pool_fwd) or (self.groups > 1 and not self.cfg.grouped_bn):
            return
        m = self.N // max(self.groups, 1)
        for pst in self.steps:
            if pst['kind'] != 'pool':
                continue
            src, dst = pst['src'], pst['dst']
            if src.root.is_input or self.act[id(src.root)].dtype != torch.float32 or self.act[id(dst.root)].dtype != torch.float32:
                continue
            prods = [o for o in self.steps if o['kind'] == 'conv' and o['dst'].root is src.root
                     and src.c0 <= o['dst'].c0 and o['dst'].c0 + o['dst'].C <= src.c0 + src.C]
            cover = sorted((o['dst'].c0, o['dst'].c0 + o['dst'].C) for o in prods)
            if not cover or cover[0][0] != src.c0 or cover[-1][1] != src.c0 + src.C or any(a[1] != b[0] for a, b in zip(cover, cover[1:])):
                continue
            ok = True
            for o in prods:
                if o.get('z') is None or o['z'].dtype != torch.float32:
                    ok = False
                    break
                zn, zc, zh, zw = o['z'].shape
                if o.get('stats') is not None or (o['plan_f'] >> 8) > 1 or o.get('lazy_to') is not None or o.get('head_lazy') or \
                        not lib.aide_bn_relu_bwd_pool_supported(m, zc, zh, zw):
                    ok = False
            if not ok:
                continue
            for o in prods:
                o['pool_out'] = dst.slice(o['dst'].c0 - src.c0, o['dst'].C)
            pst['fwd_fused'] = True

    def view(self, t, inputs=None):
        if t.root.is_input:
            x = inputs[self.g.inputs.index(t.root)]
            return x if (t.c0 == 0 and t.C == t.root.C) else x[:, t.c0:t.c0 + t.C]
        buf = self.act[id(t.root)]
        return buf if (t.c0 == 0 and t.C == t.root.C) else buf[:, t.c0:t.c0 + t.C]

    def gview(self, t):
        buf = self.grad[id(t.root)]
        return buf if (t.c0 == 0 and t.C == t.root.C) else buf[:, t.c0:t.c0 + t.C]

    def _prepare_backward(self):
        f32 = dict(device=self.dev, dtype=torch.float32)
        n, h, w = self.N, self.H, self.W
        for t in self.g.roots:
            dt = torch.bfloat16 if self.narrow_grad.get(id(t)) else torch.float32
            self.grad[id(t)] = torch.empty(n, t.C, h >> t.level, w >> t.level, device=self.dev, dtype=dt)
        for st in self.steps:
            if st['kind'] in ('conv', 'convT'):
                st['dz'] = torch.empty(st['z'].shape, device=self.dev,
                                       dtype=torch.bfloat16 if st.get('dz_bf16') else torch.float32)
        off = 0
        for st in self.steps:
            if st['kind'] in ('conv', 'convT'):
                st['wg_off'] = off
                off += (st['wg_bytes'] // 4 + 63) // 64 * 64
        self.wg_ws = torch.empty(max(off, 1), **f32)
        for st in self.steps:
            if st['kind'] in ('conv', 'convT'):
                st['wg_ws'] = self.wg_ws[st['wg_off']:st['wg_off'] + max(st['wg_bytes'] // 4, 1)]
        self.head_ws = torch.empty(max(self._max_wg // 4, 1), **f32)
        self.wg_queue = ops.new_wgrad_queue()
        sa = [st for st in self.steps if st['kind'] == 'sa']
        if sa:
            big = max(st['t1'].numel() for st in sa)
            self.sa_da, self.sa_db = torch.empty(big, **f32), torch.empty(big, **f32)
            self.sa_ws = torch.empty(max(st['gate'].numel() for st in sa) * 2 + 8, **f32)
        if self.side is None:
            self.side = _side_stream(self.dev)
        self.ev_fork, self.ev_join = ops.new_event(), ops.new_event()
        for st in self.steps:
            if st['kind'] in ('conv', 'convT'):
                st['ev'] = ops.new_event()
        cover = {id(t): _Cover() for t in self.g.roots}
        for st in reversed(self.steps):
            src = st['src']
            if src.root.is_input:
                st['src_grad'] = None
                continue
            acc, gaps = cover[id(src.root)].write(src.c0, src.c0 + src.C)
            st['src_grad'] = dict(accumulate=acc, gaps=[src.root.slice(a, b - a) for a, b in gaps])
            if st['kind'] == 'convT' and acc:
                raise NotImplementedError('ConvTranspose input with several consumers')
        for i, st in enumerate(self.steps):
            st['fold_dgrad'] = False
            sg = st.get('src_grad')
            if i == 0 or st['kind'] != 'conv' or sg is None or sg['accumulate'] or sg['gaps']:
                continue
            prod = self.steps[i - 1]
            src, dst = st['src'], prod.get('dst')
            if prod['kind'] != 'conv' or dst is None or dst.root is not src.root or (dst.c0, dst.C) != (src.c0, src.C):
                continue
            if sum(1 for o in self.steps if o.get('src') is not None and o['src'].root is src.root
                   and o['src'].c0 < src.c0 + src.C and src.c0 < o['src'].c0 + o['src'].C) != 1:
                continue
            if st['wino_d'] not in (2, 4) or (st['plan_d'] >> 8) <= 1 or prod.get('dz_bf16') or st.get('dz_bf16'):
                continue
            if self.grad[id(src.root)].dtype != torch.float32 or prod['z'].dtype != torch.float32:
                continue
            pn, pc, ph, pw = prod['z'].shape
            if not lib.aide_bn_one_pass(pn, pc, ph, pw) or (ph * pw) % 4:
                continue
            st['fold_dgrad'] = True
        for st in self.steps:
            st.pop('pool_fuse', None)
# ... 25 lines not shown
                    o['pool_fuse'] = dst.slice(o['dst'].c0 - src.c0, o['dst'].C)
                pst['bwd_fused'] = True
        if self.cfg.fuse_head_bwd:
            for hst in self.steps:
                sg = hst.get('src_grad')
                if hst['kind'] != 'head' or sg is None or sg['accumulate'] or sg['gaps']:
                    continue
                src = hst['src']
                readers = [o for o in self.steps if o.get('src') is not None and o['src'].root is src.root
                           and o['src'].c0 < src.c0 + src.C and src.c0 < o['src'].c0 + o['src'].C]
                prods = [o for o in self.steps if o['kind'] == 'conv' and o['dst'].root is src.root
                         and (o['dst'].c0, o['dst'].C) == (src.c0, src.C)]
                if len(readers) != 1 or len(prods) != 1:
                    continue
                o = prods[0]
                zn, zc, zh, zw = o['z'].shape
                if o['z'].dtype != torch.float32 or o.get('dz_bf16') or o.get('pool_fuse') is not None or \
                        not lib.aide_bn_one_pass(zn, zc, zh, zw) or (zh * zw) % 4:
                    continue
                o['head_fuse'] = hst
                hst['dgrad_fused'] = True
        self._bwd_ready = True

    def _pack_filters(self):
        convs = self._convs
        if convs is None:
            convs = self._convs = [st for st in self.steps if st['kind'] == 'conv']
            self._conv_wslots = [st['conv']._parameters for st in convs]
        ws = [d['weight'] for d in self._conv_wslots]
        key = (PARAM_EPOCH[0],) + tuple((w.data_ptr(), w._version) for w in ws)
        if key == self._pack_key:
            return None
        ptrs = tuple(k[0] for k in key[1:])
        fresh_map = self._shared['fresh']
        mine = self._pack_ids
        if mine is None:
            mine = self._pack_ids = tuple(id(st[k]) for st in convs for k in ('wf', 'wd', 'uf', 'ud') if st[k] is not None)
        fresh = frozenset(i for i in mine if fresh_map.get(i) == key)
        cached = self._pack_tabs.get((ptrs, fresh))
        if cached is None:
            split = min(4, len(convs))

            def tables(group):
                def pick(st, mode, direction):
                    t = st[_pack_slot(mode, direction)] if st['wino_' + direction] == mode else None
                    return None if (t is None or id(t) in fresh) else t
                tabs = {}
                for mode, fam in FAMILIES.items():
                    entries = [(st['conv'].weight, pick(st, mode, 'f'), pick(st, mode, 'd')) for st in group]
                    entries = [e for e in entries if e[1] is not None or e[2] is not None]
                    if entries:
                        tabs[mode] = ops._pack_table(fam, entries, self.dev)
                return tabs or None
            rest = convs[split:]
            rest_tabs = tables(rest) if rest else None
            cached = (tables(convs[:split]), rest_tabs, convs[split] if rest_tabs is not None else None)
            if len(self._pack_tabs) > 8:
                self._pack_tabs.clear()
            self._pack_tabs[(ptrs, fresh)] = cached
        first, rest, gate = cached
        self._gate_conv = gate

        def launch(tabs):
            for mode in PACK_ORDER:
                if mode in tabs:
                    ops.launch_pack_multi(FAMILIES[mode], tabs[mode])
        if fresh:
            cur = torch.cuda.current_stream()
            for s_ in self._shared['streams'] or ():
                if s_ is not None and s_ != cur:
                    cur.wait_stream(s_)
        if first is not None:
            launch(first)
        self._pack_key = key
        for i in mine:
            fresh_map[i] = key
        if rest is None:
            self._shared['streams'] = (torch.cuda.current_stream(), None)
            return None
        if self.side_fwd is None:
            pref = _preferred(self.dev)
            self.side_fwd = (self.side if self.side is not None else
                             pref['lane'] if (pref is not None and pref.get('lane') is not None) else
                             torch.cuda.Stream(device=self.dev))
            self._side_fwd_ptr = ctypes.c_void_p(self.side_fwd.cuda_stream)
            self.ev_pack_fork = ops.new_event()
        ops.order(self.ev_pack_fork, ops.stream_ptr(), self._side_fwd_ptr)
        with ops.use_stream(self._side_fwd_ptr):
            launch(rest)
        self._shared['streams'] = (torch.cuda.current_stream(), self.side_fwd)
        return gate

    def _fingerprint(self):
        fp = [self.cfg.snapshot(), FLUSH_EVERY, self.overlap]
        slots = self._fp_slots
        if slots is None:
            slots, bns = [], []
            for st in self.steps:
                if st.get('bn') is not None:
                    bns.append(st['bn'])
                for key in ('conv', 'bn', 'mod'):
                    m = st.get(key)
                    if m is None:
                        continue
                    for sub in (m.modules() if key == 'mod' else (m,)):
                        slots += [(sub._parameters, k) for k, v in sub._parameters.items() if v is not None]
                        slots += [(sub._buffers, k) for k, v in sub._buffers.items() if v is not None]
            self._fp_slots, self._fp_bns = slots, bns
        for bn in self._fp_bns:
            fp.append(bn.eps)
            fp.append(bn.momentum)
        fp += [d[k].data_ptr() for d, k in slots]
        return tuple(fp)

    def _tapeable(self):
        return self.cfg.replay and self.profiler is None and self.trace is None

    def _coef_fresh(self):
        if self.training:
            STATS_EPOCH[0] += 1
            return True
        tens = self._coef_tensors
        if tens is None:
            tens = []
            for st in self.steps:
                if st['kind'] in ('conv', 'convT'):
                    bn = st['bn']
                    tens += [st['conv'].bias, bn.weight, bn.bias, bn.running_mean, bn.running_var]
            tens = self._coef_tensors = [t for t in tens if t is not None]
            self._coef_bns = [st['bn'] for st in self.steps if st['kind'] in ('conv', 'convT')]
        self._coef_eps = [bn.eps for bn in self._coef_bns]
        key = (PARAM_EPOCH[0], STATS_EPOCH[0]) + tuple(self._coef_eps) + tuple((t.data_ptr(), t._version) for t in tens)
        self._coef_next = key
        return key == self._coef_key

    def forward(self, inputs, out):
        self.serial += 1
        gate = self._pack_filters()
        self._coef_ok = self._coef_fresh()
        self._coef_key = None
        self._forward_any(inputs, out, gate)
        if not self.training:
            self._coef_key = self._coef_next
        return out

    def _forward_any(self, inputs, out, gate):
        if not self._tapeable():
            self._tape_f = self._tape_b = None
            return self._forward_impl(inputs, out, gate, None)
        self._fp = self._fingerprint()
        dyn = list(inputs) + [out]
        key = (torch.cuda.current_stream().cuda_stream, self._fp, tuple((tuple(t.shape), t.stride()) for t in dyn))
        tp = self._tape_f
        if tp is not None and tp.key == key:
            tp.replay(dyn, skip_tags=(() if gate is not None else ('gate',)) + (('aide_bn_eval_fold',) if self._coef_ok else ()))
            return out
        tp = Tape(key)
        with tp:
            self._forward_impl(inputs, out, gate, tp)
        self._tape_f = tp.finish(dyn)
        return out

    def _forward_impl(self, inputs, out, gate, tape):
        n = self.N
        if not self.training and (tape is not None or not self._coef_ok):
            for st in self.steps:
                if st['kind'] in ('conv', 'convT'):
                    ops.bn_eval_fold(st['bn'], st['conv'].bias, st['scale'], st['shift'], st['fbias'])
        dual = self.lane_b is not None and self.cfg.dual_fwd and self.profiler is None and self.trace is None
        mp = ctypes.c_void_p(torch.cuda.current_stream().cuda_stream)
        bp = ctypes.c_void_p(self.lane_b.cuda_stream) if dual else None
        free = dual and self.cfg.free_lane
        on_b, pend = False, []
        forked = False
        touched = []
        b_reads = []
        pooled = []

        def hit(ranges, t):
            return any(r[0] is t.root and r[1] < t.c0 + t.C and t.c0 < r[1] + r[2] for r in ranges)

        def overlaps(t):
            return hit(pend, t)

        def fork_if_needed(srcs, dsts):
            nonlocal forked
            if not forked or any(hit(touched, t) for t in srcs + dsts):
                ops.order(self.ev_lane_fork, mp, bp)
                forked = True
                del touched[:]

        def main_deps(srcs, dsts):
            if any(hit(pend, t) for t in srcs + dsts) or any(hit(b_reads, t) for t in dsts):
                ops.order(self.ev_lane_join, bp, mp)
                del pend[:], b_reads[:], pooled[:]
            for e in [e for e in pooled if any(hit([e], t) for t in srcs + dsts)]:
                ops.wait(mp, e[3])
                pooled.remove(e)
        for st in self.steps:
            kind = st['kind']
            if self.trace is not None:
                self.trace('f', st)
            lane = st.get('lane', 0) if dual else 0
            if kind == 'conv' and st is self._gate_conv:
                wait = lambda: torch.cuda.current_stream().wait_stream(self.side_fwd)
                if tape is not None:
                    tape.py(wait, 'gate')
                if gate is not None:
                    wait()
                on_b = forked = False
            if free:
                srcs = [st['src']]
                dsts = [st['dst']] if st.get('dst') is not None else []
                c = st.get('lane_split') if kind == 'pool' else None
                if c and forked:
                    src, dst = st['src'], st['dst']
                    sa, da, sb, db = src.slice(0, c), dst.slice(0, c), src.slice(c, src.C - c), dst.slice(c, dst.C - c)
                    fork_if_needed([sb], [db])
                    fused = bool(st.get('fwd_fused'))
                    if not fused:
                        with ops.use_stream(bp):
                            ops.maxpool2x2_fwd(self.view(sb, inputs), self.view(db))
                    ops.record(st['ev_b'], bp)
                    pooled.append((db.root, db.c0, db.C, st['ev_b']))
                    b_reads.append((sb.root, sb.c0, sb.C))
                    main_deps([sa], [da])
                    if not fused:
                        ops.maxpool2x2_fwd(self.view(sa, inputs), self.view(da))
                    touched.extend((t.root, t.c0, t.C) for t in (sa, da))
                elif lane:
                    fork_if_needed(srcs, dsts)
                    pend.extend((t.root, t.c0, t.C) for t in dsts)
                    b_reads.extend((t.root, t.c0, t.C) for t in srcs)
                    with ops.use_stream(bp):
                        self._forward_op(st, inputs, out, self.bn_ws_b, self.sk_ws_b)
                else:
                    main_deps(srcs, dsts)
                    touched.extend((t.root, t.c0, t.C) for t in srcs + dsts)
                    self._forward_op(st, inputs, out, self.bn_ws, self.sk_ws)
                continue
            if lane and not on_b:
                ops.order(self.ev_lane_fork, mp, bp)
            on_b = bool(lane)
            if not lane and pend and (overlaps(st['src']) or (st.get('dst') is not None and overlaps(st['dst']))):
                ops.order(self.ev_lane_join, bp, mp)
                del pend[:]
            if lane:
                pend.append((st['dst'].root, st['dst'].c0, st['dst'].C))
                with ops.use_stream(bp):
                    self._forward_op(st, inputs, out, self.bn_ws_b, self.sk_ws_b)
            else:
                self._forward_op(st, inputs, out, self.bn_ws, self.sk_ws)
        if pend or pooled:
            ops.order(self.ev_lane_join, bp, mp)
        return out

    def _forward_op(self, st, inputs, out, bn_ws, sk_ws):
        kind = st['kind']
        if kind == 'conv':
            conv, bn = st['conv'], st['bn']
            x = self.view(st['src'], inputs)
            fam = FAMILIES[st['wino_f']]
            pack = st[_pack_slot(fam.mode, 'f')]
            prof = self.profiler
            if prof is not None:
                prof.begin(fam.fwd_tag, st['flops'], st['flops'] * fam.exec_frac)
            slabs = self.training and (st['plan_f'] >> 8) > 1 and \
                (st['z'].shape[2] * st['z'].shape[3]) % 4 == 0
            acc = 2 if slabs else 0
            if st.get('fold'):
                fam.conv(x, pack, st['fbias'], self.view(st['dst']), accumulate=0, plan=st['plan_f'], ws=sk_ws,
                         epi_scale=st['scale'], epi_relu=True)
                if prof is not None:
                    prof.end()
                return
            lazy = st.get('lazy_to')
            y, only4 = st['z'], {}
            if fam.mode == 4:
                in_tab = st.get('in_tab')
                only4 = dict(stats=st['stats'], in_tab=in_tab, in_group_images=(self.N // self.groups) if in_tab is not None else 0)
                if lazy is not None:
                    y = self.view(st['dst'])
            fam.conv(x, pack, conv.bias, y, accumulate=acc, plan=st['plan_f'], ws=sk_ws, **only4)
            if prof is not None:
                prof.end()
            if st.get('head_lazy'):
                zn, zc, zh, zw = st['z'].shape
                ops.bn_finalize_groups(zn, 1, zc, zh, zw, bn, st['stats'], st['stats_parts'], st['stats_parts'], conv.bias,
                                       st['mean'], st['rstd'], st['scale'], st['shift'], st['head_tab'], 0)
            elif lazy is not None:
                zz = self.view(st['dst'])
                ops.bn_finalize_groups(self.N // self.groups, self.groups, zz.shape[1], zz.shape[2], zz.shape[3], bn,
                                       st['stats'], st['stats_parts'] // self.groups, st['stats_parts'], conv.bias,
                                       st['mean'], st['rstd'], st['scale'], st['shift'], lazy['in_tab'], st['tab_c0'])
            else:
                self._bn_apply(st, bn, conv.bias if slabs else None, (st['plan_f'] >> 8) if slabs else 0, bn_ws, sk_ws)
        elif kind == 'convT':
            conv, bn = st['conv'], st['bn']
            ops.convT2x2_fwd(self.view(st['src'], inputs), conv.weight, conv.bias, st['z'])
            self._bn_apply(st, bn, None, 0, bn_ws, sk_ws)
        elif kind == 'pool':
            if not (st.get('fwd_fused') and self.training):
                ops.maxpool2x2_fwd(self.view(st['src'], inputs), self.view(st['dst']))
        elif kind == 'up':
            ops.upsample2x_fwd(self.view(st['src'], inputs), self.view(st['dst']))
        elif kind == 'head':
            conv = st['conv']
            lp = st.get('lazy_prod')
            if lp is not None:
                ops.head1x1_fwd_bn(lp['z'], lp['scale'], lp['shift'], conv.weight.view(conv.out_channels, -1), conv.bias, out)
# ... 263 lines not shown
                                   self.gview(st['src']), accumulate=sg['accumulate'])
        elif kind == 'up':
            if sg is not None:
                ops.upsample2x_bwd(self.gview(st['dst']), self.gview(st['src']),
                                   accumulate=sg['accumulate'])




def _has_param_hooks(params):
    for p in params:
        if p._backward_hooks or getattr(p, '_post_accumulate_grad_hooks', None):
            return True
    return False


import sys as _sys


def _max_refs(views):
    m = 0
    for v in views:
        m = max(m, _sys.getrefcount(v))
    return m


_REF_BASE = _max_refs([object()])


_STORAGE_USES = getattr(torch._C, '_storage_Use_Count', None)


def _storage_uses(t):
    return _STORAGE_USES(t.untyped_storage()._cdata) if _STORAGE_USES is not None else -1


def _views_held_elsewhere(views, arena=None, base_uses=-1):
    if _max_refs(views) > _REF_BASE:
        return True
    return arena is not None and base_uses >= 0 and _storage_uses(arena) > base_uses


class _NetFunction(torch.autograd.Function):

    @staticmethod
    def forward(ctx, engine, n_inputs, direct, *tensors):
        inputs = tensors[:n_inputs]
        plan = engine.plan_for(inputs)
        plan.profiler = engine.profiler
        k = engine.num_classes
        n, _, h, w = inputs[0].shape
        out = torch.empty(n, k, h, w, device=inputs[0].device, dtype=torch.float32)
        plan.forward(inputs, out)
        cur = torch.cuda.current_stream(inputs[0].device)
        for x in inputs:
            x.record_stream(cur)
        ctx.engine, ctx.plan, ctx.serial, ctx.inputs, ctx.direct = engine, plan, plan.serial, inputs, direct
        ctx.ntensors = len(tensors)
        return out

    @staticmethod
    def backward(ctx, dlogits):
        eng, plan = ctx.engine, ctx.plan
        if ctx.serial != plan.serial or eng.plans.get(plan.key) is not plan:
            raise RuntimeError('aide_amd: backward() after a newer forward() of the same module at the same input shape '
                               '— its activations were overwritten (the engine keeps one set per module and shape)')
        if not plan.training:
            raise RuntimeError('aide_amd: backward through an eval-mode forward is not supported')
        dlogits = dlogits.contiguous()
        dlogits.record_stream(torch.cuda.current_stream(dlogits.device))
        params = eng.params
        mode = 0
        if ctx.direct:
            arena, views = eng.grad_arena(dlogits.device)
            have = [p.grad for p in params]
            if all(g is None for g in have):
                mode = 1
                if _views_held_elsewhere(views, arena, eng._arena_uses):
                    arena, views = eng.grad_arena(dlogits.device, fresh=True)
            else:
                base = arena.data_ptr()
                if all(g is not None and g.data_ptr() == base + 4 * o and g.dtype == torch.float32
                       for g, o in zip(have, eng.offsets)):
                    mode = 2
                else:
                    mode = 3
        flat = arena if mode == 1 else torch.empty(eng.flat_numel, device=dlogits.device, dtype=torch.float32)
        eng.side_stream = plan.side if (plan._bwd_ready and plan.overlap) else None
        if not plan._bwd_ready:
            plan._prepare_backward()
            eng.side_stream = plan.side if plan.overlap else None
        if eng.before_backward is not None:
            eng.before_backward(flat)
        plan.backward(ctx.inputs, dlogits, flat, eng.offsets, eng.after_backward_op)
        if eng.grad_hook is not None:
            eng.grad_hook(flat)
        if mode == 0:
            grads = tuple(flat[o:o + p.numel()].view(p.shape) for o, p in zip(eng.offsets, params))
            return (None, None, None) + (None,) * len(ctx.inputs) + grads
        if mode == 1:
            for p, v in zip(params, views):
                if p.requires_grad:
                    p.grad = v
        elif mode == 2:
            arena.add_(flat)
        else:
            for p, o, g in zip(params, eng.offsets, have):
                if not p.requires_grad:
                    continue
                v = flat[o:o + p.numel()].view(p.shape)
                if g is None:
                    p.grad = v
                else:
                    g.add_(v)
        z = eng._anchor_zero
        if z is None or z.device != dlogits.device:
            z = eng._anchor_zero = torch.zeros(1, device=dlogits.device)
        return (None,) * (3 + ctx.ntensors - 1) + (z,)


class Engine(object):
    MAX_PLANS = 6

    def __init__(self, module, build_graph, num_classes):
        if not 1 <= int(num_classes) <= 8:
            raise NotImplementedError('aide_amd: num_classes must be 1 .. 8, got %r' % (num_classes,))
        self.module, self.build_graph, self.num_classes = module, build_graph, num_classes
        self.plans = {}
        self._shared_packs = dict(buf={}, fresh={}, streams=None)
        self.params = None
        self.grad_hook = None
        self.after_backward_op = None
        self.profiler = None
        self.before_backward = None
        self.side_stream = None
        self.graph = None
        self._precision = 'fp32'
        self.config = EngineConfig(self._config_changed)
        self.pending_stream = None
        self._arena = self._views = self._anchor = self._anchor_zero = None
        self._arena_uses = -1
        self._pslots = None

    def _join_pending(self):
        s = self.pending_stream
        if s is not None:
            cur = torch.cuda.current_stream(s.device)
            if cur != s:
                cur.wait_stream(s)
                self.pending_stream = None

    def _config_changed(self):
        self.plans = {}
        self._shared_packs = dict(buf={}, fresh={}, streams=None)

    def grad_arena(self, device, fresh=False):
        a = self._arena
        if fresh or a is None or a.numel() != self.flat_numel or a.device != device:
            a = self._arena = torch.zeros(self.flat_numel, device=device, dtype=torch.float32)
            self._views = [a[o:o + p.numel()].view(p.shape) for o, p in zip(self.offsets, self.params)]
            self._arena_uses = _storage_uses(a)
        return a, self._views

    @property
    def precision(self):
        return self._precision

    @precision.setter
    def precision(self, value):
        if value not in PRECISIONS:
            raise ValueError('aide_amd: precision must be one of %s (got %r)' % (PRECISIONS, value))
        if value != self._precision:
            self._precision = value
            self.plans = {}
            self._shared_packs = dict(buf={}, fresh={}, streams=None)

    def _refresh_params(self):
        slots = self._pslots
        if slots is not None and self.params is not None and all(d.get(k) is p for d, k, p in slots):
            return
        params = list(self.module.parameters())
        self._pslots = [(m._parameters, k, p) for m in self.module.modules() for k, p in m._parameters.items()
                        if p is not None]
        if self.params is None or len(params) != len(self.params) or \
                any(a is not b for a, b in zip(params, self.params)):
            self.params = params
            self.graph = self.build_graph()
            index = {id(p): i for i, p in enumerate(params)}
            order = []
            for op in reversed(self.graph.ops):
                for key in ('conv', 'bn', 'mod'):
                    m = op.get(key)
                    if m is not None:
                        order += [index[id(p)] for p in m.parameters()]
            seen = set(order)
            assert len(seen) == len(order), 'a parameter is owned by two graph ops'
            order += [i for i in range(len(params)) if i not in seen]
            self.offsets, off = [0] * len(params), 0
            for i in order:
                self.offsets[i] = off
                off += (params[i].numel() + 3) // 4 * 4
            self.flat_numel = off
            self.plans = {}
            self._shared_packs = dict(buf={}, fresh={}, streams=None)
            self._arena = self._views = None

    @staticmethod
    def invalidate_coefficients():
        STATS_EPOCH[0] += 1

    def plan_for(self, inputs, groups=1):
        self._refresh_params()
        x = inputs[0]
        n, _, h, w = x.shape
        if h % 16 or w % 16:
            raise RuntimeError('aide_amd: H and W must be multiples of 16 (got %dx%d)' % (h, w))
        key = (n, h, w, x.device.index, bool(self.module.training), self._precision, groups)
        plan = self.plans.get(key)
        if plan is None:
            for op in self.graph.ops:
                for t in (op.get('src'), op.get('dst')):
                    if t is not None and t.C * (h >> t.level) * (w >> t.level) * 4 >= 2 ** 31:
                        raise RuntimeError('aide_amd: %dx%d is too large: %d channels of %s exceed the 2 GiB per-image '
                                           'operand limit of the kernels' % (h, w, t.C, t.name))
            plan = Plan(self.graph, self.params, n, h, w, x.device, bool(self.module.training), self._precision,
                        groups, shared=self._shared_packs if self.config.shared_packs else None, cfg=self.config)
            plan.key = key
            self.plans[key] = plan
            while len(self.plans) > self.MAX_PLANS:
                self.plans.pop(next(iter(self.plans)))
        else:
            self.plans[key] = self.plans.pop(key)
        return plan

    def run_groups(self, input_groups):
        self._join_pending()
        groups = len(input_groups)
        nin = len(input_groups[0])
        ins = []
        for k in range(nin):
            xs = [grp[k] for grp in input_groups]
            for x in xs:
                if not isinstance(x, torch.Tensor) or not x.is_cuda or x.dtype != torch.float32 or x.dim() != 4:
                    raise RuntimeError('aide_amd: inputs must be fp32 NCHW tensors on a HIP device')
                if x.shape != xs[0].shape:
                    raise RuntimeError('aide_amd: grouped forward needs equal input shapes')
            ins.append(torch.cat([x.detach() for x in xs], 0))
        with torch.no_grad():
            plan = self.plan_for(ins, groups)
            plan.profiler = self.profiler
            n, _, h, w = ins[0].shape
            out = torch.empty(n, self.num_classes, h, w, device=ins[0].device, dtype=torch.float32)
            plan.forward(ins, out)
        m = n // groups
        return [out[g * m:(g + 1) * m] for g in range(groups)]

    def run(self, *inputs):
        self._join_pending()
        ins = []
        for x in inputs:
            if not isinstance(x, torch.Tensor) or not x.is_cuda:
                raise RuntimeError('aide_amd models run on a HIP device only (input on %s); there is no '
                                   'CPU fallback — use the reference for CPU runs'
                                   % (x.device if isinstance(x, torch.Tensor) else type(x)))
            if x.dtype != torch.float32 or x.dim() != 4:
                raise RuntimeError('aide_amd: inputs must be fp32 NCHW tensors')
            ins.append(x.contiguous())
        self._refresh_params()
        for p in self.params:
            if not p.is_cuda:
                raise RuntimeError('aide_amd: module parameters are on %s; call .to(device) first' % p.device)
        if self.config.direct_grads and torch.is_grad_enabled() and any(p.requires_grad for p in self.params) and \
                not _has_param_hooks(self.params):
            if self._anchor is None or self._anchor.device != ins[0].device:
                self._anchor = torch.zeros(1, device=ins[0].device, requires_grad=True)
            self._anchor.grad = None
            return _NetFunction.apply(self, len(ins), True, *(tuple(ins) + (self._anchor,)))
        return _NetFunction.apply(self, len(ins), False, *(tuple(ins) + tuple(self.params)))
```

aide_amd/ops.py:

```python
import collections
import ctypes
import struct

import torch

from ._lib import lib, check


_STREAM = [None]


def stream_ptr():
    if _STREAM[0] is not None:
        return _STREAM[0]
    return ctypes.c_void_p(torch.cuda.current_stream().cuda_stream)


class use_stream(object):

    def __init__(self, sptr):
        self.sptr = sptr if isinstance(sptr, ctypes.c_void_p) else ctypes.c_void_p(sptr)

    def __enter__(self):
        self.prev = _STREAM[0]
# ... 488 lines not shown


def bf16_pack_alloc(cout, cin, device):
    return torch.empty(lib.aide_conv3x3_bf16_pack_elems(cout, cin), device=device, dtype=torch.int16)


def bf16_pack_table(entries, device):
    return _pack_table(FAMILIES[BF16], entries, device)


def bf16_pack(w, need_dgrad=True):
    return _pack_one(FAMILIES[BF16], w, need_dgrad)


def conv3x3_bf16(x, u, bias, y, accumulate=False, splitk=-1, ws=None, plan=None):
    xp, xbs = planes(x, bf16_ok=True)
    yp, ybs = planes(y, bf16_ok=True)
    n, cin, h, w = x.shape
    cout = y.shape[1]
    assert u.dtype == torch.int16 and u.numel() == lib.aide_conv3x3_bf16_pack_elems(cout, cin)
    splitk, ws = _splitk_ws(FAMILIES[BF16], x, cout, splitk, plan, ws)
    check(lib.aide_conv3x3_bf16_mixed(xp, int(is_bf16(x)), xbs, ptr(u), ptr(bias), yp, int(is_bf16(y)), ybs, n, cin, h,
                                      w, cout, int(accumulate), splitk, ptr(ws), stream_ptr()), 'conv3x3_bf16')
    return y


def wgrad_bf16_supported(co, ci, h, w):
    return bool(lib.aide_conv3x3_wgrad_bf16_supported(co, ci, h, w))


def conv3x3_wgrad_bf16(dz, a, dw, ws=None, queue=None, co_blocks=0):
    dzp, dzbs = planes(dz, bf16_ok=True)
    ap, abs_ = planes(a, bf16_ok=True)
    n, co, h, w = dz.shape
    ci = a.shape[1]
    assert tuple(dw.shape) == (co, ci, 3, 3) and dw.is_contiguous()
    if ws is None:
        ws = torch.empty(lib.aide_conv3x3_wgrad_bf16_ws_bytes(n, co, ci, h, w, co_blocks) // 4, device=dz.device,
                         dtype=torch.float32)
    check(lib.aide_conv3x3_wgrad_bf16_mixed(dzp, int(is_bf16(dz)), dzbs, ap, int(is_bf16(a)), abs_, ptr(dw), n, co, ci,
                                            h, w, ptr(ws), co_blocks, _qh(queue), stream_ptr()), 'conv3x3_wgrad_bf16')
    return dw


def wgrad_wino4_supported(co, ci, h, w):
    return bool(lib.aide_conv3x3_wgrad_wino4_supported(co, ci, h, w))


def conv3x3_wgrad_wino4(dz, a, dw, ws=None, target_wgs=0, queue=None):
    dzp, dzbs = planes(dz)
    ap, abs_ = planes(a)
    n, co, h, w = dz.shape
    ci = a.shape[1]
    if ws is None:
        ws = torch.empty(lib.aide_conv3x3_wgrad_wino4_ws_bytes_t(n, co, ci, h, w, target_wgs) // 4, device=dz.device,
                         dtype=torch.float32)
    elif target_wgs and ws.numel() * 4 < lib.load().aide_conv3x3_wgrad_wino4_ws_bytes_t(n, co, ci, h, w, target_wgs):
        raise RuntimeError('aide_amd: weight-gradient workspace too small for %d workgroups' % target_wgs)
    check(lib.aide_conv3x3_wgrad_wino4_t(dzp, dzbs, ap, abs_, ptr(dw), n, co, ci, h, w, ptr(ws), target_wgs, _qh(queue),
                                         stream_ptr()), 'conv3x3_wgrad_wino4')
    return dw


def wgrad_wino_supported(co, ci, h, w):
    return bool(lib.aide_conv3x3_wgrad_wino_supported(co, ci, h, w))


def conv3x3_wgrad_wino(dz, a, dw, ws=None, queue=None):
    dp, dbs = planes(dz)
    ap, abs_ = planes(a)
    n, co, h, w = dz.shape
    ci = a.shape[1]
    assert tuple(dw.shape) == (co, ci, 3, 3) and dw.is_contiguous()
    if ws is None:
        ws = torch.empty(lib.aide_conv3x3_wgrad_wino_ws_bytes(n, co, ci, h, w) // 4, device=dz.device,
                         dtype=torch.float32)
    check(lib.aide_conv3x3_wgrad_wino(dp, dbs, ap, abs_, ptr(dw), n, co, ci, h, w, ptr(ws), _qh(queue), stream_ptr()),
          'conv3x3_wgrad_wino')
    return dw


ConvFamily = collections.namedtuple('ConvFamily', 'mode fwd_tag wgrad_tag exec_frac supported wgrad_supported plan pack_alloc '
                                    'pack_blocks pack_padded pack_multi conv wgrad wgrad_ws_bytes')


def _f32_pack(rows, taps):
    return lambda cin, cout, device: torch.empty(rows(cin), taps, cout, device=device, dtype=torch.float32)


FAMILIES = {
    0: ConvFamily(
        0, 'conv3x3_mfma_kernel', 'conv3x3_wgrad_kernel', 1.0,
        supported=lambda cin, h, w, cout: True, wgrad_supported=lambda co, ci, h, w: True,
        plan=lambda n, cin, h, w, cout: lib.aide_conv3x3_plan(n, cin, h, w, cout),
        pack_alloc=_f32_pack(lambda cin: pad_to(cin, conv_chunk(cin)), 9),
        pack_blocks=lambda co, ci, uf, ud: (sum(t.numel() for t in (uf, ud) if t is not None) + 255) // 256,
        pack_padded=True, pack_multi='conv3x3_pack_weights_multi', conv=conv3x3_igemm, wgrad=conv3x3_wgrad,
        wgrad_ws_bytes=lambda n, co, ci, h, w: lib.aide_conv3x3_wgrad_ws_bytes(n, co, ci, h, w)),
    2: ConvFamily(
        2, 'conv3x3_wino_kernel', 'conv3x3_wgrad_wino_kernel', 16.0 / 36.0,
        supported=wino_supported, wgrad_supported=wgrad_wino_supported,
        plan=lambda n, cin, h, w, cout: lib.aide_conv3x3_wino_splitk(n, cin, h, w, cout) << 8,
        pack_alloc=_f32_pack(lambda cin: pad_to(cin, 8), 16),
        pack_blocks=lambda co, ci, uf, ud: lib.aide_conv3x3_wino_pack_blocks(co, ci),
        pack_padded=True, pack_multi='conv3x3_wino_pack_multi', conv=conv3x3_wino, wgrad=conv3x3_wgrad_wino,
        wgrad_ws_bytes=lambda n, co, ci, h, w: lib.aide_conv3x3_wgrad_wino_ws_bytes(n, co, ci, h, w)),
    4: ConvFamily(
        4, 'conv3x3_wino4_kernel', 'conv3x3_wgrad4_kernel', 36.0 / 144.0,
        supported=wino4_supported, wgrad_supported=wgrad_wino4_supported,
        plan=lambda n, cin, h, w, cout: lib.aide_conv3x3_wino4_splitk(n, cin, h, w, cout) << 8,
        pack_alloc=_f32_pack(lambda cin: cin, 36),
        pack_blocks=lambda co, ci, uf, ud: lib.aide_conv3x3_wino4_pack_blocks(co, ci),
        pack_padded=False, pack_multi='conv3x3_wino4_pack_multi', conv=conv3x3_wino4, wgrad=conv3x3_wgrad_wino4,
        wgrad_ws_bytes=lambda n, co, ci, h, w, target_wgs=0:
            lib.aide_conv3x3_wgrad_wino4_ws_bytes_t(n, co, ci, h, w, target_wgs)),
    BF16: ConvFamily(
        BF16, 'conv3x3_bf16_kernel', 'conv3x3_wgrad_bf16_kernel', 1.0,
        supported=bf16_supported, wgrad_supported=wgrad_bf16_supported,
        plan=lambda n, cin, h, w, cout: lib.aide_conv3x3_bf16_splitk(n, cin, h, w, cout) << 8,
        pack_alloc=lambda cin, cout, device: bf16_pack_alloc(cout, cin, device),
        pack_blocks=lambda co, ci, uf, ud: lib.aide_conv3x3_bf16_pack_blocks(co, ci),
        pack_padded=False, pack_multi='conv3x3_bf16_pack_multi', conv=conv3x3_bf16, wgrad=conv3x3_wgrad_bf16,
        wgrad_ws_bytes=lambda n, co, ci, h, w, co_blocks=0:
            lib.aide_conv3x3_wgrad_bf16_ws_bytes(n, co, ci, h, w, co_blocks)),
}


def _splitk_ws(fam, x, cout, splitk, plan, ws):
    n, cin, h, w = x.shape
    if plan is not None:
        splitk = plan >> 8
    elif splitk < 0:
        splitk = fam.plan(n, cin, h, w, cout) >> 8
    if splitk > 1 and ws is None:
        ws = torch.empty(lib.aide_conv3x3_ws_bytes(n, h, w, cout, splitk) // 4, device=x.device, dtype=torch.float32)
    return splitk, ws


def _pack_table(fam, entries, device):
    rec, start = b'', 0
    for w, uf, ud in entries:
        co, ci = w.shape[0], w.shape[1]
        rows = [t.shape[0] if (fam.pack_padded and t is not None) else 0 for t in (uf, ud)]
        rec += struct.pack('<QQQiiiiq', w.data_ptr(), uf.data_ptr() if uf is not None else 0,
                           ud.data_ptr() if ud is not None else 0, co, ci, rows[0], rows[1], start)
        start += fam.pack_blocks(co, ci, uf, ud)
    return torch.frombuffer(bytearray(rec), dtype=torch.uint8).to(device), len(entries), start


def launch_pack_multi(fam, tab):
    check(getattr(lib, 'aide_' + fam.pack_multi)(ptr(tab[0]), tab[1], tab[2], stream_ptr()), fam.pack_multi)


def _pack_one(fam, w, need_dgrad):
    _req(w)
    co, ci = w.shape[0], w.shape[1]
    uf = fam.pack_alloc(ci, co, w.device)
    ud = fam.pack_alloc(co, ci, w.device) if need_dgrad else None
    launch_pack_multi(fam, _pack_table(fam, [(w, uf, ud)], w.device))
    return uf, ud


def _dense(t):
    _req(t)
    if not t.is_contiguous():
        raise RuntimeError('aide_amd: dense contiguous tensor expected')
    return ptr(t)


def pwconv_fwd(x, w, b, y):
    xp, xbs = planes(x)
    yp, ybs = planes(y)
    n, c, h, wd = x.shape
    r = y.shape[1]
    assert w.numel() == r * c
    check(lib.aide_pwconv_fwd(xp, xbs, ptr(w), ptr(b), yp, ybs, n, c, r, h * wd, stream_ptr()), 'pwconv_fwd')
    return y


def pwconv_dgrad(dt, w, dx, gate=None, dout=None, accumulate=False):
    tp, tbs = planes(dt)
    xp, xbs = planes(dx)
    n, c, h, wd = dx.shape
    r = dt.shape[1]
    assert w.numel() == r * c
    dp, dbs = planes(dout) if dout is not None else (ctypes.c_void_p(0), 0)
    check(lib.aide_pwconv_dgrad(tp, tbs, ptr(w), ptr(gate), dp, dbs, xp, xbs, n, c, r, h * wd, int(accumulate),
                                stream_ptr()), 'pwconv_dgrad')
    return dx


def pwconv_wgrad(dt, x, dw, db):
    tp, tbs = planes(dt)
    xp, xbs = planes(x)
    n, c, h, wd = x.shape
    r = dt.shape[1]
    assert dw.numel() == r * c
    check(lib.aide_pwconv_wgrad(tp, tbs, xp, xbs, ptr(dw), ptr(db), n, c, r, h * wd, stream_ptr()), 'pwconv_wgrad')


def dconv_small(x, w, b, y, dilation, transposed=False):
    n, cx, h, wd = x.shape
    cout, cin = w.shape[0], w.shape[1]
    assert (cx, y.shape[1]) == ((cout, cin) if transposed else (cin, cout))
    check(lib.aide_dconv3x3_small(_dense(x), _dense(w), ptr(b), _dense(y), n, cin, cout, h, wd, dilation,
                                  int(transposed), stream_ptr()), 'dconv3x3_small')
    return y


def dconv_small_wgrad(dy, x, dw, db, dilation):
    n, cout, h, wd = dy.shape
    cin = x.shape[1]
    check(lib.aide_dconv3x3_small_wgrad(_dense(dy), _dense(x), ptr(dw), ptr(db), n, cout, cin, h, wd, dilation,
                                        stream_ptr()), 'dconv3x3_small_wgrad')


def sa_gate_fwd(t4, bn, training, stat, gate):
    check(lib.aide_sa_gate_fwd(_dense(t4), ptr(bn.weight), ptr(bn.bias), ptr(bn.running_mean), ptr(bn.running_var),
                               ptr(bn.num_batches_tracked), float(bn.eps), float(bn.momentum), int(training),
                               ptr(stat), _dense(gate), t4.numel(), stream_ptr()), 'sa_gate_fwd')


def sa_mul(gate, y, out):
    yp, ybs = planes(y)
    op_, obs = planes(out)
    n, c, h, wd = y.shape
    check(lib.aide_sa_mul(_dense(gate), yp, ybs, op_, obs, n, c, h * wd, stream_ptr()), 'sa_mul')


def sa_gate_bwd(dout, y, gate, t4, stat, gamma, dgamma, dbeta, dt4, ws):
    dp, dbs = planes(dout)
    yp, ybs = planes(y)
    n, c, h, wd = y.shape
    assert ws.numel() >= n * h * wd + 4
    check(lib.aide_sa_gate_bwd(dp, dbs, yp, ybs, _dense(gate), _dense(t4), ptr(stat), ptr(gamma), ptr(dgamma),
                               ptr(dbeta), _dense(dt4), n, c, h * wd, ptr(ws), stream_ptr()), 'sa_gate_bwd')
```

aide_amd/optim.py:

```python
import ctypes

import torch

from . import engine
from ._lib import lib, check
from .ops import stream_ptr, ptr


class Adam(torch.optim.Optimizer):
    def __init__(self, params, lr=1e-3, betas=(0.9, 0.999), eps=1e-8, weight_decay=0, amsgrad=False):
        if lr < 0 or eps < 0 or not 0 <= betas[0] < 1 or not 0 <= betas[1] < 1:
            raise ValueError('invalid Adam hyper-parameters')
        super(Adam, self).__init__(params, dict(lr=lr, betas=betas, eps=eps, weight_decay=weight_decay,
                                                amsgrad=amsgrad))
        self._tables = {}
        self._gtabs = {}
        self._fast = {}

    def load_state_dict(self, state_dict):
        super(Adam, self).load_state_dict(state_dict)
        self._tables = {}
        self._fast = {}

    def add_param_group(self, param_group):
        super(Adam, self).add_param_group(param_group)
        self._fast = {}

    def zero_grad(self, set_to_none=True):
        if not set_to_none:
            return super(Adam, self).zero_grad(set_to_none=False)
        for group in self.param_groups:
            for p in group['params']:
                p.grad = None

    def _launch(self, tab, gtab, n, group, step):
        if tab['total_blocks'] == 0:
            return
        b1, b2 = group['betas']
        check(lib.aide_adam_amsgrad_multi(ptr(tab['p']), ptr(gtab), ptr(tab['m']), ptr(tab['v']),
                                          ptr(tab['vmax']), ptr(tab['sizes']), ptr(tab['starts']),
                                          n, tab['total_blocks'], float(group['lr']), float(b1),
                                          float(b2), float(group['eps']), float(group['weight_decay']),
                                          int(bool(group['amsgrad'])), step, stream_ptr()), 'adam')

    def _static_table(self, slot, plist):
        st = [self.state[p] for p in plist]
        key = tuple((p.data_ptr(), p.numel(), s['exp_avg'].data_ptr(), s['exp_avg_sq'].data_ptr(),
                     s['max_exp_avg_sq'].data_ptr() if 'max_exp_avg_sq' in s else 0) for p, s in zip(plist, st))
        tab = self._tables.get(slot)
        if tab is not None and tab['key'] == key:
            return tab
        dev = plist[0].device
        sizes = [p.numel() for p in plist]
        starts, acc = [], 0
        for s in sizes:
            starts.append(acc)
            acc += (s + 1023) // 1024

        def table(vals):
            return torch.tensor(vals, dtype=torch.int64).to(dev)
        tab = dict(key=key, total_blocks=acc,
                   p=table([k[0] for k in key]), m=table([k[2] for k in key]), v=table([k[3] for k in key]),
                   vmax=table([k[4] for k in key]), sizes=table(sizes), starts=table(starts))
        self._tables[slot] = tab
        return tab

    def _grad_table(self, slot, grads):
        gkey = tuple(g.data_ptr() for g in grads)
        cached = self._gtabs.get(slot)
        if cached is not None and cached[0] == gkey:
            return gkey, cached[1]
        gtab = torch.tensor(gkey, dtype=torch.int64).to(grads[0].device, non_blocking=True)
        self._gtabs[slot] = (gkey, gtab)
        return gkey, gtab

    @staticmethod
    def _state_unchanged(fast):
        step = fast['step']
        for st, m, v, vm in fast['moments']:
            if st['step'] is not step or st['exp_avg'] is not m or st['exp_avg_sq'] is not v or \
                    st.get('max_exp_avg_sq') is not vm:
                return False
        return True

    @torch.no_grad()
    def step(self, closure=None):
        loss = None
        if closure is not None:
            with torch.enable_grad():
                loss = closure()
        keep = []
        for gi, group in enumerate(self.param_groups):
            fast = self._fast.get(gi)
            if fast is not None:
                params = group['params']
                grads = [p.grad for p in params]
                if fast['params'] is params and len(params) == fast['n'] and all(g is not None for g in grads) and \
                        tuple(g.data_ptr() for g in grads) == fast['gkey'] and \
                        tuple(p.data_ptr() for p in params) == fast['pkey'] and \
                        bool(group['amsgrad']) == fast['amsgrad'] and self._state_unchanged(fast):
                    step = fast['step'] = fast['step'] + 1
                    for st in fast['states']:
                        st['step'] = step
                    self._launch(fast['tab'], fast['gtab'], fast['n'], group, step)
                    keep.append(fast['gtab'])
                    continue
                self._fast.pop(gi, None)
            plist = [p for p in group['params'] if p.grad is not None]
            if not plist:
                continue
            for p in plist:
                if not p.is_cuda or p.dtype != torch.float32 or not p.is_contiguous():
                    raise RuntimeError('aide_amd.optim.Adam: parameters must be contiguous fp32 HIP tensors')
                st = self.state[p]
                if len(st) and group['amsgrad'] and 'max_exp_avg_sq' not in st:
                    st['max_exp_avg_sq'] = st['exp_avg_sq'].clone()
                if len(st) == 0:
                    st['step'] = 0
                    st['exp_avg'] = torch.zeros_like(p)
                    st['exp_avg_sq'] = torch.zeros_like(p)
                    if group['amsgrad']:
                        st['max_exp_avg_sq'] = torch.zeros_like(p)
            buckets = {}
            for p in plist:
                buckets.setdefault(int(self.state[p]['step']), []).append(p)
            for j, (prev, ps) in enumerate(sorted(buckets.items())):
                slot = (gi, j)
                tab = self._static_table(slot, ps)
                grads = [p.grad if p.grad.is_contiguous() else p.grad.contiguous() for p in ps]
                gkey, gtab = self._grad_table(slot, grads)
                step = prev + 1
                for p in ps:
                    self.state[p]['step'] = step
                self._launch(tab, gtab, len(ps), group, step)
                keep.append(gtab)
                keep.extend(g for g, p in zip(grads, ps) if g is not p.grad)
            for slot in [s for s in self._tables if s[0] == gi and s[1] >= len(buckets)]:
                self._tables.pop(slot)
                self._gtabs.pop(slot, None)
            if len(buckets) == 1 and len(plist) == len(group['params']) and all(g is p.grad for g, p in zip(grads, plist)):
                states = [self.state[p] for p in plist]
                self._fast[gi] = dict(params=group['params'], n=len(plist), gkey=gkey,
                                      pkey=tuple(p.data_ptr() for p in plist), amsgrad=bool(group['amsgrad']),
                                      step=step, states=states, tab=tab, gtab=gtab,
                                      moments=[(s, s['exp_avg'], s['exp_avg_sq'], s.get('max_exp_avg_sq'))
                                               for s in states])
        self._keep = keep
        engine.PARAM_EPOCH[0] += 1
        return loss
```

include/aide_hip.h:

```cpp
#ifndef AIDE_HIP_H
#define AIDE_HIP_H
#include <stddef.h>
#include <stdint.h>

#ifdef __cplusplus
extern "C" {
#endif

typedef struct ihipStream_t* aide_stream_t;

int aide_conv3x3_chunk(int Cin);
int aide_conv3x3_pack_weights(const float* w , float* wf ,
                              float* wd , int Co, int Ci, int ci_pad,
                              int co_pad, aide_stream_t stream);
int aide_conv3x3_pack_weights_multi(const void* descs, int n, int64_t total_blocks, aide_stream_t stream);
int aide_conv3x3_plan(int N, int Cin, int H, int W, int Cout);
size_t aide_conv3x3_ws_bytes(int N, int H, int W, int Cout, int splitk);
int aide_conv3x3_igemm(const float* x, int64_t x_bs, const float* wp, int ldw, const float* bias,
                       float* y, int64_t y_bs, int N, int Cin, int H, int W, int Cout, int accumulate,
                       int plan, float* ws, const float* epi_scale, int epi_relu,
                       aide_stream_t stream);
int aide_conv3x3_wino_supported(int Cin, int H, int W, int Cout);
int aide_conv3x3_wino_splitk(int N, int Cin, int H, int W, int Cout);
int aide_conv3x3_wino4_supported(int Cin, int H, int W, int Cout);
// ... 188 lines not shown
int aide_head1x1_fwd_mixed(const void* x, int x_bf16, int64_t x_bs, const float* w, const float* b, float* y,
                           int64_t y_bs, int N, int C, int K, int H, int W, aide_stream_t stream);
int aide_head1x1_bwd_mixed(const float* dy, int64_t dy_bs, const void* x, int x_bf16, int64_t x_bs, const float* w,
                           void* dx, int dx_bf16, int64_t dx_bs, float* dw, float* db, int N, int C, int K, int H, int W,
                           void* ws, aide_stream_t stream);
int aide_seg_loss_blocks(int HW);
size_t aide_seg_loss_ws_bytes(int N, int HW);
int aide_seg_stats(const float* logits, int64_t l_bs, const long long* targets, int64_t t_bs, float w0,
                   float w1, int ignore_index, const float* pseudo, int64_t p_bs, const float* wmap,
                   int64_t w_bs, int N, int HW, double* partials, aide_stream_t stream);
int aide_seg_loss_finalize(const double* partials, int N, int HW, int reduction, float w_ce, float w_dice,
                           float smooth, double* stats, float* out, float* per_image, long long* idx,
                           float* coef, float* hard_dice, aide_stream_t stream);
int aide_coteach_finalize(const double* partials1, const double* partials2, int N, int HW, int variant,
                          int keep, float w_ce, float w_dice, float smooth, float rate, float w_seg,
                          float w_cor, double* stats1, double* stats2, float* loss, float* per_image1,
                          float* per_image2, long long* idx1, long long* idx2, float* coef1, float* coef2,
                          float* hard_dice, aide_stream_t stream);
int aide_seg_loss_bwd(const float* logits, int64_t l_bs, const long long* targets, int64_t t_bs, float w0,
                      float w1, int ignore_index, const float* pseudo, int64_t p_bs, const float* wmap,
                      int64_t w_bs, int N, int HW, const double* stats, const float* coef, float smooth,
                      const float* gout, int g_stride, float* dlogits, int64_t d_bs, aide_stream_t stream);
int aide_ce_map(const float* logits, int64_t l_bs, const long long* targets, int64_t t_bs, float w0,
                float w1, int ignore_index, int N, int HW, float* out, const float* gout, float* dlogits,
                int64_t d_bs, aide_stream_t stream);
int aide_mse_map(const float* logits, int64_t l_bs, const float* target, int64_t q_bs, int N, int HW,
                 float* out, const float* gout, float* dlogits, int64_t d_bs, aide_stream_t stream);
int aide_pseudo_label(const float* const* logits , int K,
                      int64_t l_bs, int N, int HW, float temperature, float* pl, float* wm,
                      aide_stream_t stream);

int aide_seg_max_classes(void);
int aide_seg_stats_mc(const float* logits, int64_t l_bs, const long long* targets, int64_t t_bs,
                      const float* class_w , int C, int ignore_index, const float* pseudo, int64_t p_bs,
                      const float* wmap, int64_t w_bs, int N, int HW, double* partials, aide_stream_t stream);
int aide_seg_loss_bwd_mc(const float* logits, int64_t l_bs, const long long* targets, int64_t t_bs,
                         const float* class_w , int C, int ignore_index, const float* pseudo, int64_t p_bs,
                         const float* wmap, int64_t w_bs, int N, int HW, const double* stats, const float* coef,
                         float smooth, const float* gout, int g_stride, float* dlogits, int64_t d_bs,
                         aide_stream_t stream);
int aide_coteach_finalize_mc(const double* partials1, const double* partials2, int N, int HW, int C, int variant,
                             int keep, float w_ce, float w_dice, float smooth, float rate, float w_seg,
                             float w_cor, double* stats1, double* stats2, float* loss, float* per_image1,
                             float* per_image2, long long* idx1, long long* idx2, float* coef1, float* coef2,
                             float* hard_dice, aide_stream_t stream);
int aide_ce_map_mc(const float* logits, int64_t l_bs, const long long* targets, int64_t t_bs,
                   const float* class_w , int C, int ignore_index, int N, int HW, float* out,
                   const float* gout, float* dlogits, int64_t d_bs, aide_stream_t stream);
int aide_mse_map_mc(const float* logits, int64_t l_bs, const float* target, int64_t q_bs, int C, int N, int HW,
                    float* out, const float* gout, float* dlogits, int64_t d_bs, aide_stream_t stream);
int aide_label_map_mc(const float* logits, int64_t l_bs, int C, int N, int HW, long long* labels,
                      aide_stream_t stream);
int aide_pseudo_label_mc(const float* const* logits , int K, int C,
                         int64_t l_bs, int N, int HW, float temperature, float* pl, float* wm,
                         aide_stream_t stream);
int aide_kl_map_mc(const float* z1, int64_t b1, const float* z2, int64_t b2, int C, int N, int HW, float* out,
                   const float* gout, float* g1, int64_t gb1, float* g2, int64_t gb2, aide_stream_t stream);
int aide_region_ce_fwd_mc(const float* z, int64_t zb, const long long* t, int64_t tb, int C, int N, int H, int W,
                          int ignore_index, float* loss, unsigned* aux, aide_stream_t stream);
int aide_region_ce_bwd_mc(const float* z, int64_t zb, const unsigned* aux, const unsigned char* mask, const float* coeff,
                          int C, int N, int H, int W, float* dz, int64_t db, aide_stream_t stream);
int aide_droppixel_map_mc(const float* z1, int64_t b1, const float* z2, int64_t b2, const long long* t, int64_t tb,
                          const long long* idx, int ndrop, int C, int HW, int which, int ignore_index, float* v,
                          aide_stream_t stream);
int aide_droppixel_bwd_mc(const float* z1, int64_t b1, const float* z2, int64_t b2, const long long* t, int64_t tb,
                          const long long* idx, int ndrop, int C, int HW, int which, int ignore_index,
                          const unsigned char* mask, const float* coeff, float* g1, float* g2, aide_stream_t stream);
size_t aide_dice_terms_mc_ws_bytes(int N, int HW, int C);
int aide_dice_terms_mc_fwd(const float* x, int64_t x_bs, const float* t, int64_t t_bs, int N, int HW, int C,
                           const float* class_w , float smooth, int reduction, double* ws,
                           float* per_image, float* out, aide_stream_t stream);
int aide_dice_terms_mc_bwd(const float* x, int64_t x_bs, const float* t, int64_t t_bs, int N, int HW, int C,
                           const float* class_w , float smooth, int reduction, const double* ws,
                           const float* g, float* dx, int64_t dx_bs, aide_stream_t stream);

int aide_kl_map(const float* z1, int64_t b1, const float* z2, int64_t b2, int N, int HW, float* out,
                const float* gout, float* g1, int64_t gb1, float* g2, int64_t gb2, aide_stream_t stream);
int aide_region_ce_fwd(const float* z, int64_t zb, const long long* t, int64_t tb, int N, int H, int W,
                       int ignore_index, float* loss, unsigned char* aux, aide_stream_t stream);
int aide_region_ce_bwd(const float* z, int64_t zb, const unsigned char* aux, const unsigned char* mask,
                       const float* coeff, int N, int H, int W, float* dz, int64_t db, aide_stream_t stream);
int aide_region_ce_fwd_win(const float* z, int64_t zb, const long long* t, int64_t tb, int C, int N, int H, int W, int KH,
                           int KW, int ignore_index, float* loss, int* aux, aide_stream_t stream);
int aide_region_ce_bwd_win(const float* z, int64_t zb, const int* aux, const unsigned char* mask, const float* coeff, int C,
                           int N, int H, int W, int KH, int KW, float* dz, int64_t db, aide_stream_t stream);
int aide_select_smallest(const float* sel_vals, const float* sum_vals, int64_t seg_stride, int nseg, int M,
                         int64_t k_host, double rr, const long long* k_in, int only_positive, unsigned char* mask,
                         double* sums, long long* ks, aide_stream_t stream);
int aide_droppixel_map(const float* z1, int64_t b1, const float* z2, int64_t b2, const long long* t, int64_t tb,
                       const long long* idx, int ndrop, int HW, int which, float* v, aide_stream_t stream);
int aide_droppixel_bwd(const float* z1, int64_t b1, const float* z2, int64_t b2, const long long* t, int64_t tb,
                       const long long* idx, int ndrop, int HW, int which, const unsigned char* mask,
                       const float* coeff, float* g1, float* g2, aide_stream_t stream);

int aide_pixelcoreg_map(const float* z1, const float* z2, const float* z3, const long long* t, int64_t tb, int N,
                        int HW, float kd, float* key, float* val, float* tf, aide_stream_t stream);
int aide_pixelcoreg_bwd(const float* z1, const float* z2, const float* z3, const long long* t, int64_t tb, int N,
                        int HW, float kd, const unsigned char* mask, const float* coeff, float* g1, float* g2,
                        float* g3, aide_stream_t stream);

int aide_label_map(const float* logits, int64_t l_bs, int N, int HW, long long* labels, aide_stream_t stream);

size_t aide_lcc3d_ws_bytes(int64_t nvox);
int aide_keep_largest_cc3d(const long long* v, int64_t d0, int64_t d1, int64_t d2, int64_t s0, int64_t s1, int64_t s2,
                           unsigned char* out, void* ws, aide_stream_t stream);
int aide_case_confusion(const void* p, int p_u8, int64_t p_s0, int64_t p_s1, int64_t p_s2, const void* t, int t_u8,
                        int64_t t_s0, int64_t t_s1, int64_t t_s2, int64_t d0, int64_t d1, int64_t d2, long long* out,
                        aide_stream_t stream);

size_t aide_lcc3d_batched_ws_bytes(int64_t nvox_total, int64_t K);
int aide_keep_largest_cc3d_batched(const long long* v, const long long* slice_start, int64_t K, int64_t S_total, int64_t H,
                                   int64_t W, unsigned char* out, void* ws, aide_stream_t stream);
int aide_case_confusion_batched(const unsigned char* p, const unsigned char* target, const long long* slice_start, int64_t K,
                                int64_t S_total, int64_t H, int64_t W, int match, long long* out, aide_stream_t stream);

int aide_label_refresh_select(const long long* sums, const unsigned char* labelled, int64_t K, int64_t n_select, float* dice,
                              int* rank, unsigned char* selected, aide_stream_t stream);
int aide_label_bank_update(const unsigned char* pred, const unsigned char* selected, const long long* slice_start, int64_t K,
                           int64_t S_total, int64_t H, int64_t W, int scale, unsigned char* bank_plane, aide_stream_t stream);
int aide_label_bank_targets(const unsigned char* bank_plane, int64_t S_total, int64_t H, int64_t W, const long long* slice_idx,
                            int64_t N, const int* palette, int npal, long long* out, aide_stream_t stream);

int aide_image_eval_logits(const float* logits, int64_t l_bs, const unsigned char* score_rows, const unsigned char* gate,
                           int64_t N, int64_t H, int64_t W, int64_t k0, int64_t K, unsigned char* pred, long long* sums,
                           aide_stream_t stream);
int aide_image_eval_labels(const void* labels, int is_u8, const unsigned char* score_rows, const unsigned char* gate, int64_t N,
                           int64_t H, int64_t W, int64_t k0, int64_t K, unsigned char* pred, long long* sums,
                           aide_stream_t stream);
int aide_image_refresh_select(const long long* sums, const unsigned char* labelled, int64_t K, int64_t n_select, float* dice,
                              int* rank, unsigned char* written, aide_stream_t stream);
int aide_image_bank_update(const unsigned char* pred, const unsigned char* written, int64_t K, int64_t H, int64_t W, int scale,
                           unsigned char* plane, aide_stream_t stream);
int aide_image_bank_targets(const unsigned char* plane, int64_t K, int64_t H, int64_t W, const long long* image_idx, int64_t N,
                            const unsigned char* gate, long long* out, aide_stream_t stream);

int aide_mc_counts_logits(const float* logits, int64_t l_bs, const void* target, int t_kind, int64_t t_bs, int C, int64_t N,
                          int64_t HW, long long* counts, aide_stream_t stream);
int aide_mc_counts_labels(const void* p, int p_u8, int64_t p_s0, int64_t p_s1, int64_t p_s2, const void* t, int t_u8,
                          int64_t t_s0, int64_t t_s1, int64_t t_s2, int64_t d0, int64_t d1, int64_t d2, int C,
                          long long* counts, aide_stream_t stream);
int aide_mc_metrics_accumulate(const long long* counts, int64_t N, int C, int64_t HW, void* acc, aide_stream_t stream);

size_t aide_loader_aug_ws_bytes(int nplanes, int S);
int aide_loader_aug(const void* src, const int* desc, const int* tab, const double* par, const float* norm, int N, int M,
                    int S, int augno, int out_u8, void* out, void* ws, aide_stream_t stream);
int aide_loader_mask_onehot(const void* src, const int* desc, const int* tab, const int* palette, int nplanes, int S,
                            int npal, long long* out, aide_stream_t stream);

int aide_adam_amsgrad_multi(float* const* p, const float* const* g, float* const* m, float* const* v,
                            float* const* vmax, const int64_t* sizes, const int64_t* block_start,
                            int ntensors, int64_t total_blocks, float lr, float beta1, float beta2,
                            float eps, float weight_decay, int amsgrad, int64_t step,
                            aide_stream_t stream);

#ifdef __cplusplus
}
#endif
#endif
```

Measured before the change: 645.9 images/sec.

## Fuse Adam update with Winograd weight packing for 3x3 conv params

Adds an adam_pack kernel that applies the AMSGrad Adam update to 3x3 conv weights tile by tile and immediately writes the Winograd-transformed forward/dgrad packs from the updated tile in shared memory. The shared pack logic moves into a common header. The optimizer splits params into packed-linked and plain groups and marks packs as refreshed, so the separate pack pass before the next forward can be skipped. This removes a re-read of the weights and a kernel launch per step, at the cost of more complex cache invalidation between the optimizer and the engine.

```diff
diff --git a/aide_amd/build.py b/aide_amd/build.py
--- a/aide_amd/build.py
+++ b/aide_amd/build.py
@@ -38,7 +38,8 @@
         sp = os.path.join(CSRC, src)
         op = os.path.join(OBJ, src.replace('.hip', '.o'))
         stamp = op + '.sha1'
-        dg = _digest([sp, common])
+        own = [os.path.join(CSRC, h) for h in ('wino_pack.h',) if '#include "%s"' % h in open(sp).read()]
+        dg = _digest([sp, common] + own)
         if not force and os.path.exists(op) and os.path.exists(stamp) and open(stamp).read() == dg:
             return op, False
         cmd = [hipcc] + FLAGS + ['-c', sp, '-o', op]
diff --git a/aide_amd/csrc/conv3x3_wino4.hip b/aide_amd/csrc/conv3x3_wino4.hip
--- a/aide_amd/csrc/conv3x3_wino4.hip
+++ b/aide_amd/csrc/conv3x3_wino4.hip
@@ -1,4 +1,5 @@
 #include "common.h"
+#include "wino_pack.h"
 #include <stdlib.h>
 #include <type_traits>
 
@@ -32,9 +33,6 @@
 constexpr int F4_SET = F4_RAW + F4_V;
 constexpr int F4_LDS = 2 * F4_SET > 4 * 128 * 64 ? 2 * F4_SET : 4 * 128 * 64;
 
-__host__ __device__ constexpr int f4_pos(int q, int b) {
-    return 6 * (q / 3) + ((q % 3) == 0 ? 1 + b : (q % 3) == 1 ? 3 + b : 5 * b);
-}
 __host__ __device__ constexpr int f4_slot(int c) { return c == 0 ? 4 : c == 5 ? 5 : c - 1; }
 
 __device__ __forceinline__ void bt6(float d0, float d1, float d2, float d3, float d4, float d5, float* o, int st) {
@@ -419,90 +417,14 @@
     }
 }
 
-__device__ __forceinline__ void wino4_g(const float g[9], float u[36]) {
-    float t[18];
-#pragma unroll
-    for (int c = 0; c < 3; ++c) {
-        const float g0 = g[c], g1 = g[3 + c], g2 = g[6 + c];
-        const float s = g0 + g2;
-        t[c] = 0.25f * g0;
-        t[3 + c] = (-1.f / 6.f) * (s + g1);
-        t[6 + c] = (-1.f / 6.f) * (s - g1);
-        const float q = __builtin_fmaf(4.f, g2, g0);
-        t[9 + c] = (1.f / 24.f) * (q + 2.f * g1);
-        t[12 + c] = (1.f / 24.f) * (q - 2.f * g1);
-        t[15 + c] = g2;
-    }
-#pragma unroll
-    for (int r = 0; r < 6; ++r) {
-        const float a0 = t[r * 3], a1 = t[r * 3 + 1], a2 = t[r * 3 + 2];
-        const float s = a0 + a2, q = __builtin_fmaf(4.f, a2, a0);
-        u[r * 6] = 0.25f * a0;
-        u[r * 6 + 1] = (-1.f / 6.f) * (s + a1);
-        u[r * 6 + 2] = (-1.f / 6.f) * (s - a1);
-        u[r * 6 + 3] = (1.f / 24.f) * (q + 2.f * a1);
-        u[r * 6 + 4] = (1.f / 24.f) * (q - 2.f * a1);
-        u[r * 6 + 5] = a2;
-    }
-}
-
-struct W4PackDesc {
-    const float* w; float* uf; float* ud;
-    int Co, Ci, pad0, pad1;
-    long block_start;
-};
-
-constexpr int P4_T = 32;
-__global__ __launch_bounds__(128) void wino4_pack_multi_kernel(const W4PackDesc* __restrict__ descs, int n, long total_blocks) {
-    __shared__ __attribute__((aligned(16))) float ot[36 * 128];
+__global__ __launch_bounds__(P4_THREADS) void wino4_pack_multi_kernel(const W4PackDesc* __restrict__ descs, int n, long total_blocks) {
+    __shared__ __attribute__((aligned(16))) float ot[P4_OT];
     for (long blk = blockIdx.x; blk < total_blocks; blk += gridDim.x) {
-    int lo = 0, hi = n - 1;
-    while (lo < hi) {
-        const int mid = (lo + hi + 1) >> 1;
-        if (descs[mid].block_start <= blk) lo = mid; else hi = mid - 1;
-    }
-    const W4PackDesc d = descs[lo];
-    const int tid = threadIdx.x;
-    const int tiles_ci = (d.Ci + P4_T - 1) / P4_T;
-    const int tb = (int)(blk - d.block_start);
-    const int co0 = (tb / tiles_ci) * P4_T, ci0 = (tb % tiles_ci) * P4_T;
-    const int nci = min(P4_T, d.Ci - ci0);
-    float g[9], u[36];
-    const int lo2 = tid & 3, hi5 = tid >> 2;
-    for (int grp = 0; grp < 16; ++grp) {
-        const bool fwd = grp < 8;
-        const int q = grp & 7;
-        float* dst = fwd ? d.uf : d.ud;
-        if (dst == nullptr) continue;
-        const int co = fwd ? hi5 : 4 * q + lo2, ci = fwd ? 4 * q + lo2 : hi5;
-        const bool live = fwd ? (ci0 + 4 * q < d.Ci) : (co0 + 4 * q < d.Co);
-        if (!live) continue;
-        {
-            const bool in = co0 + co < d.Co && ci < nci;
-            const float* wp = d.w + ((long)(co0 + co) * d.Ci + ci0 + ci) * 9;
-#pragma unroll
-            for (int t = 0; t < 9; ++t) g[t] = in ? wp[fwd ? t : 8 - t] : 0.f;
-        }
-        wino4_g(g, u);
-        const int otid = (lo2 >> 1) * 64 + hi5 * 2 + (lo2 & 1);
-#pragma unroll
-        for (int p = 0; p < 36; ++p) ot[p * 128 + otid] = u[p];
-        __syncthreads();
-        const int C = fwd ? d.Co : d.Ci, c0 = fwd ? co0 : ci0;
-        const long gbase = (long)((fwd ? ci0 : co0) / 4 + q) * 18;
-        const int nrow = min(P4_T, C - c0);
-#pragma unroll
-        for (int k = 0; k < 9; ++k) {
-            const int f = tid + k * 128, pq = f >> 6, hh = (f >> 5) & 1, row = f & 31;
-            if (row < nrow) {
-                const float* o0 = ot + f4_pos(pq, 0) * 128 + hh * 64 + row * 2;
-                const float* o1 = ot + f4_pos(pq, 1) * 128 + hh * 64 + row * 2;
-                *reinterpret_cast<f32x4*>(dst + (((gbase + pq) * 2 + hh) * C + c0 + row) * 4) =
-                    f32x4{o0[0], o0[1], o1[0], o1[1]};
-            }
-        }
-        __syncthreads();
-    }
+        const W4PackDesc d = descs[pack_desc_of(descs, n, blk)];
+        const int tiles_ci = (d.Ci + P4_T - 1) / P4_T;
+        const int tb = (int)(blk - d.block_start);
+        const int co0 = (tb / tiles_ci) * P4_T, ci0 = (tb % tiles_ci) * P4_T;
+        wino4_pack_tile(d, co0, ci0, ot, [&](int co, int ci) { return d.w + ((long)(co0 + co) * d.Ci + ci0 + ci) * 9; });
     }
 }
 
@@ -548,7 +470,7 @@
     if (!descs || n <= 0 || total_blocks <= 0) return AIDE_ERR_ARG;
     static_assert(sizeof(W4PackDesc) == 48, "descriptor layout");
     const long grid = total_blocks;
-    AIDE_LAUNCH_TIMED(AIDE_KT_OTHER, 0.0, wino4_pack_multi_kernel, dim3((unsigned)grid), dim3(128), 0, stream,
+    AIDE_LAUNCH_TIMED(AIDE_KT_OTHER, 0.0, wino4_pack_multi_kernel, dim3((unsigned)grid), dim3(P4_THREADS), 0, stream,
                        (const W4PackDesc*)descs, n, (long)total_blocks);
     return aide_launch_status();
 }
diff --git a/aide_amd/csrc/conv3x3_winograd.hip b/aide_amd/csrc/conv3x3_winograd.hip
--- a/aide_amd/csrc/conv3x3_winograd.hip
+++ b/aide_amd/csrc/conv3x3_winograd.hip
@@ -1,4 +1,5 @@
 #include "common.h"
+#include "wino_pack.h"
 
 namespace {
 
@@ -270,73 +271,14 @@
     *reinterpret_cast<f32x4*>(p) = v;
 }
 
-struct WinoPackDesc {
-    const float* w; float* uf; float* ud;
-    int Co, Ci, ci_pad, co_pad;
-    long block_start;
-};
-
-__device__ __forceinline__ void wino_g(const float g[9], float u[16]) {
-    float t[12];
-#pragma unroll
-    for (int c = 0; c < 3; ++c) {
-        const float g0 = g[c], g1 = g[3 + c], g2 = g[6 + c];
-        t[c] = g0; t[3 + c] = 0.5f * (g0 + g1 + g2); t[6 + c] = 0.5f * (g0 - g1 + g2); t[9 + c] = g2;
-    }
-#pragma unroll
-    for (int r = 0; r < 4; ++r) {
-        const float a0 = t[r * 3], a1 = t[r * 3 + 1], a2 = t[r * 3 + 2];
-        u[r * 4] = a0; u[r * 4 + 1] = 0.5f * (a0 + a1 + a2); u[r * 4 + 2] = 0.5f * (a0 - a1 + a2); u[r * 4 + 3] = a2;
-    }
-}
-
-constexpr int WP_T = 32;
-__global__ __launch_bounds__(256) void wino_pack_multi_kernel(const WinoPackDesc* __restrict__ descs, int n) {
-    __shared__ __attribute__((aligned(16))) float ot[16 * 256];
+__global__ __launch_bounds__(WP_THREADS) void wino_pack_multi_kernel(const WinoPackDesc* __restrict__ descs, int n) {
+    __shared__ __attribute__((aligned(16))) float ot[WP_OT];
     const long blk = blockIdx.x;
-    int lo = 0, hi = n - 1;
-    while (lo < hi) {
-        const int mid = (lo + hi + 1) >> 1;
-        if (descs[mid].block_start <= blk) lo = mid; else hi = mid - 1;
-    }
-    const WinoPackDesc d = descs[lo];
-    const int tid = threadIdx.x;
+    const WinoPackDesc d = descs[pack_desc_of(descs, n, blk)];
     const int tiles_ci = (d.Ci + WP_T - 1) / WP_T;
     const int tb = (int)(blk - d.block_start);
     const int co0 = (tb / tiles_ci) * WP_T, ci0 = (tb % tiles_ci) * WP_T;
-    const int nci = min(WP_T, d.Ci - ci0);
-    float g[9], u[16];
-    const int lo3 = tid & 7, hi5 = tid >> 3;
-    for (int grp = 0; grp < 8; ++grp) {
-        const bool fwd = grp < 4;
-        const int q = grp & 3;
-        float* dst = fwd ? d.uf : d.ud;
-        if (dst == nullptr) continue;
-        const int co = fwd ? hi5 : 8 * q + lo3, ci = fwd ? 8 * q + lo3 : hi5;
-        const bool live = fwd ? (ci0 + 8 * q < d.ci_pad) : (co0 + 8 * q < d.co_pad);
-        if (!live) continue;
-        {
-            const bool in = co0 + co < d.Co && ci < nci;
-            const float* wp = d.w + ((long)(co0 + co) * d.Ci + ci0 + ci) * 9;
-#pragma unroll
-            for (int t = 0; t < 9; ++t) g[t] = in ? wp[fwd ? t : 8 - t] : 0.f;
-        }
-        wino_g(g, u);
-#pragma unroll
-        for (int p = 0; p < 16; ++p) ot[p * 256 + tid] = u[p];
-        __syncthreads();
-        const int C = fwd ? d.Co : d.Ci, c0 = fwd ? co0 : ci0;
-        const long gbase = (long)((fwd ? ci0 : co0) / 8 + q) * 16;
-        const int nrun = min(WP_T, C - c0) * 8;
-#pragma unroll
-        for (int k = 0; k < 4; ++k) {
-            const int f = tid + k * 256, p = f >> 6, x4 = (f & 63) * 4;
-            if (x4 < nrun)
-                *reinterpret_cast<f32x4*>(dst + ((gbase + p) * C + c0) * 8 + x4) =
-                    *reinterpret_cast<const f32x4*>(ot + p * 256 + x4);
-        }
-        __syncthreads();
-    }
+    wino_pack_tile(d, co0, ci0, ot, [&](int co, int ci) { return d.w + ((long)(co0 + co) * d.Ci + ci0 + ci) * 9; });
 }
 
 }
@@ -362,7 +304,7 @@
 int aide_conv3x3_wino_pack_multi(const void* descs, int n, int64_t total_blocks, hipStream_t stream) {
     if (!descs || n <= 0 || total_blocks <= 0) return AIDE_ERR_ARG;
     static_assert(sizeof(WinoPackDesc) == 48, "descriptor layout");
-    AIDE_LAUNCH_TIMED(AIDE_KT_OTHER, 0.0, wino_pack_multi_kernel, dim3((unsigned)total_blocks), dim3(256), 0, stream,
+    AIDE_LAUNCH_TIMED(AIDE_KT_OTHER, 0.0, wino_pack_multi_kernel, dim3((unsigned)total_blocks), dim3(WP_THREADS), 0, stream,
                        (const WinoPackDesc*)descs, n);
     return aide_launch_status();
 }
diff --git a/aide_amd/csrc/head_adam.hip b/aide_amd/csrc/head_adam.hip
--- a/aide_amd/csrc/head_adam.hip
+++ b/aide_amd/csrc/head_adam.hip
@@ -1,4 +1,5 @@
 #include "common.h"
+#include "wino_pack.h"
 
 namespace {
 
@@ -147,6 +148,20 @@
     int amsgrad;
 };
 
+template <class A>
+__device__ __forceinline__ float adam_update(const A& a, float pi, float gi, float& mi, float& vi, float& vmax) {
+    if (a.weight_decay != 0.f) gi = __builtin_fmaf(a.weight_decay, pi, gi);
+    mi = __builtin_fmaf(a.beta1, mi, (1.f - a.beta1) * gi);
+    float bv = a.beta2 * vi, gg = (1.f - a.beta2) * gi * gi;
+    asm("" : "+v"(bv));
+    asm("" : "+v"(gg));
+    vi = bv + gg;
+    float vhat = vi;
+    if (a.amsgrad) { vhat = fmaxf(vmax, vi); vmax = vhat; }
+    const float denom = sqrtf(vhat) / a.bc2_sqrt + a.eps;
+    return __builtin_fmaf(-(a.lr / a.bc1), mi / denom, pi);
+}
+
 __global__ __launch_bounds__(256) void adam_kernel(const AdamArgs a) {
     const long blk = blockIdx.x;
     int lo = 0, hi = a.ntensors - 1;
@@ -163,17 +178,98 @@
     for (int k = 0; k < 4; ++k) {
         const long i = base + k * 256 + threadIdx.x;
         if (i < n) {
-            float gi = g[i];
-            const float pi = p[i];
-            if (a.weight_decay != 0.f) gi += a.weight_decay * pi;
-            const float mi = a.beta1 * m[i] + (1.f - a.beta1) * gi;
-            const float vi = a.beta2 * v[i] + (1.f - a.beta2) * gi * gi;
+            float mi = m[i], vi = v[i], vmi = a.amsgrad ? vm[i] : 0.f;
+            const float pn = adam_update(a, p[i], g[i], mi, vi, vmi);
             m[i] = mi; v[i] = vi;
-            float vhat = vi;
-            if (a.amsgrad) { vhat = fmaxf(vm[i], vi); vm[i] = vhat; }
-            const float denom = sqrtf(vhat) / a.bc2_sqrt + a.eps;
-            p[i] = pi - (a.lr / a.bc1) * (mi / denom);
-        }
+            if (a.amsgrad) vm[i] = vmi;
+            p[i] = pn;
+        }
+    }
+}
+
+struct AdamPackDesc {
+    float* p; float* m; float* v; float* vmax;
+    float* uf; float* ud;
+    int Co, Ci, pad0, pad1;
+    long block_start;
+};
+struct AdamCoef { float lr, beta1, beta2, eps, weight_decay, bc1, bc2_sqrt; int amsgrad; };
+
+constexpr int AP_ROW = 32 * 9 + 1;
+
+template <int FAM>
+__global__ __launch_bounds__(FAM == 4 ? P4_THREADS : WP_THREADS)
+void adam_pack_kernel(const AdamPackDesc* __restrict__ descs, const float* const* __restrict__ grads, int n, const AdamCoef a) {
+    constexpr int NT = FAM == 4 ? P4_THREADS : WP_THREADS;
+    constexpr int U = 3;
+    __shared__ float tile[32 * AP_ROW];
+    __shared__ __attribute__((aligned(16))) float ot[FAM == 4 ? P4_OT : WP_OT];
+    const long blk = blockIdx.x;
+    const int di = pack_desc_of(descs, n, blk);
+    const AdamPackDesc d = descs[di];
+    const float* __restrict__ g = grads[di];
+    const int tid = threadIdx.x;
+    const int tiles_ci = (d.Ci + 31) / 32;
+    const int tb = (int)(blk - d.block_start);
+    const int co0 = (tb / tiles_ci) * 32, ci0 = (tb % tiles_ci) * 32;
+    const int nco = min(32, d.Co - co0), rowlen = min(32, d.Ci - ci0) * 9;
+    const long row = (long)d.Ci * 9, base = (long)co0 * row + (long)ci0 * 9;
+    const bool vec = (d.Ci & 3) == 0 &&
+        ((((uintptr_t)d.p | (uintptr_t)g | (uintptr_t)d.m | (uintptr_t)d.v | (a.amsgrad ? (uintptr_t)d.vmax : 0)) & 15) == 0);
+    if (vec) {
+        const int cpr = rowlen >> 2, total = nco * cpr;
+        for (int f0 = tid; f0 < total; f0 += U * NT) {
+            f32x4 pv[U], gv[U], mv[U], vv[U], xv[U];
+            long off[U];
+            int lds[U];
+#pragma unroll
+            for (int u = 0; u < U; ++u) {
+                const int f = f0 + u * NT;
+                if (f < total) {
+                    const int r = f / cpr, c = (f - r * cpr) * 4;
+                    off[u] = base + r * row + c;
+                    lds[u] = r * AP_ROW + c;
+                    pv[u] = ld4(d.p + off[u]); gv[u] = ld4(g + off[u]); mv[u] = ld4(d.m + off[u]); vv[u] = ld4(d.v + off[u]);
+                    xv[u] = a.amsgrad ? ld4(d.vmax + off[u]) : f32x4{0.f, 0.f, 0.f, 0.f};
+                }
+            }
+#pragma unroll
+            for (int u = 0; u < U; ++u) {
+                if (f0 + u * NT < total) {
+#pragma unroll
+                    for (int e = 0; e < 4; ++e) {
+                        float mi = mv[u][e], vi = vv[u][e], xi = xv[u][e];
+                        pv[u][e] = adam_update(a, pv[u][e], gv[u][e], mi, vi, xi);
+                        mv[u][e] = mi; vv[u][e] = vi; xv[u][e] = xi;
+                        tile[lds[u] + e] = pv[u][e];
+                    }
+                    st4(d.m + off[u], mv[u]); st4(d.v + off[u], vv[u]);
+                    if (a.amsgrad) st4(d.vmax + off[u], xv[u]);
+                    st4(d.p + off[u], pv[u]);
+                }
+            }
+        }
+    } else {
+        const int total = nco * rowlen;
+        for (int f = tid; f < total; f += NT) {
+            const int r = f / rowlen, c = f - r * rowlen;
+            const long i = base + r * row + c;
+            float mi = d.m[i], vi = d.v[i], xi = a.amsgrad ? d.vmax[i] : 0.f;
+            const float pn = adam_update(a, d.p[i], g[i], mi, vi, xi);
+            d.m[i] = mi; d.v[i] = vi;
+            if (a.amsgrad) d.vmax[i] = xi;
+            d.p[i] = pn;
+            tile[r * AP_ROW + c] = pn;
+        }
+    }
+    __syncthreads();
+    const auto taps = [&](int co, int ci) { return tile + (co * AP_ROW + ci * 9); };
+    if constexpr (FAM == 4) {
+        const W4PackDesc pd{d.p, d.uf, d.ud, d.Co, d.Ci, d.pad0, d.pad1, d.block_start};
+        wino4_pack_tile(pd, co0, ci0, ot, taps);
+    } else {
+        const WinoPackDesc pd{d.p, d.uf, d.ud, d.Co, d.Ci, d.pad0, d.pad1, d.block_start};
+        wino_pack_tile(pd, co0, ci0, ot, taps);
     }
 }
 
@@ -273,4 +369,23 @@
     return aide_launch_status();
 }
 
-}
+int aide_adam_pack_multi(const void* descs, const float* const* grads, int n, int64_t total_blocks, int family, float lr,
+                         float beta1, float beta2, float eps, float weight_decay, int amsgrad, int64_t step,
+                         hipStream_t stream) {
+    if (!descs || !grads || n <= 0 || total_blocks <= 0 || step < 1 || (family != 4 && family != 2)) return AIDE_ERR_ARG;
+    static_assert(sizeof(AdamPackDesc) == 72, "descriptor layout");
+    AdamCoef a;
+    a.lr = lr; a.beta1 = beta1; a.beta2 = beta2; a.eps = eps; a.weight_decay = weight_decay;
+    a.bc1 = (float)(1.0 - pow((double)beta1, (double)step));
+    a.bc2_sqrt = (float)sqrt(1.0 - pow((double)beta2, (double)step));
+    a.amsgrad = amsgrad;
+    if (family == 4)
+        AIDE_LAUNCH_TIMED(AIDE_KT_OTHER, 0.0, adam_pack_kernel<4>, dim3((unsigned)total_blocks), dim3(P4_THREADS), 0, stream,
+                          (const AdamPackDesc*)descs, grads, n, a);
+    else
+        AIDE_LAUNCH_TIMED(AIDE_KT_OTHER, 0.0, adam_pack_kernel<2>, dim3((unsigned)total_blocks), dim3(WP_THREADS), 0, stream,
+                          (const AdamPackDesc*)descs, grads, n, a);
+    return aide_launch_status();
+}
+
+}
diff --git a/aide_amd/csrc/wino_pack.h b/aide_amd/csrc/wino_pack.h
--- /dev/null
+++ b/aide_amd/csrc/wino_pack.h
@@ -0,0 +1,155 @@
+#pragma once
+#include "common.h"
+
+namespace {
+
+__host__ __device__ constexpr int f4_pos(int q, int b) {
+    return 6 * (q / 3) + ((q % 3) == 0 ? 1 + b : (q % 3) == 1 ? 3 + b : 5 * b);
+}
+
+__device__ __forceinline__ void wino4_g(const float g[9], float u[36]) {
+    float t[18];
+#pragma unroll
+    for (int c = 0; c < 3; ++c) {
+        const float g0 = g[c], g1 = g[3 + c], g2 = g[6 + c];
+        const float s = g0 + g2;
+        t[c] = 0.25f * g0;
+        t[3 + c] = (-1.f / 6.f) * (s + g1);
+        t[6 + c] = (-1.f / 6.f) * (s - g1);
+        const float q = __builtin_fmaf(4.f, g2, g0);
+        t[9 + c] = (1.f / 24.f) * (q + 2.f * g1);
+        t[12 + c] = (1.f / 24.f) * (q - 2.f * g1);
+        t[15 + c] = g2;
+    }
+#pragma unroll
+    for (int r = 0; r < 6; ++r) {
+        const float a0 = t[r * 3], a1 = t[r * 3 + 1], a2 = t[r * 3 + 2];
+        const float s = a0 + a2, q = __builtin_fmaf(4.f, a2, a0);
+        u[r * 6] = 0.25f * a0;
+        u[r * 6 + 1] = (-1.f / 6.f) * (s + a1);
+        u[r * 6 + 2] = (-1.f / 6.f) * (s - a1);
+        u[r * 6 + 3] = (1.f / 24.f) * (q + 2.f * a1);
+        u[r * 6 + 4] = (1.f / 24.f) * (q - 2.f * a1);
+        u[r * 6 + 5] = a2;
+    }
+}
+
+struct W4PackDesc {
+    const float* w; float* uf; float* ud;
+    int Co, Ci, pad0, pad1;
+    long block_start;
+};
+
+constexpr int P4_T = 32, P4_THREADS = 128, P4_OT = 36 * 128;
+template <class Taps>
+__device__ __forceinline__ void wino4_pack_tile(const W4PackDesc& d, int co0, int ci0, float* ot, Taps&& taps) {
+    const int tid = threadIdx.x;
+    const int nci = min(P4_T, d.Ci - ci0);
+    float g[9], u[36];
+    const int lo2 = tid & 3, hi5 = tid >> 2;
+    for (int grp = 0; grp < 16; ++grp) {
+        const bool fwd = grp < 8;
+        const int q = grp & 7;
+        float* dst = fwd ? d.uf : d.ud;
+        if (dst == nullptr) continue;
+        const int co = fwd ? hi5 : 4 * q + lo2, ci = fwd ? 4 * q + lo2 : hi5;
+        const bool live = fwd ? (ci0 + 4 * q < d.Ci) : (co0 + 4 * q < d.Co);
+        if (!live) continue;
+        {
+            const bool in = co0 + co < d.Co && ci < nci;
+            const float* wp = taps(co, ci);
+#pragma unroll
+            for (int t = 0; t < 9; ++t) g[t] = in ? wp[fwd ? t : 8 - t] : 0.f;
+        }
+        wino4_g(g, u);
+        const int otid = (lo2 >> 1) * 64 + hi5 * 2 + (lo2 & 1);
+#pragma unroll
+        for (int p = 0; p < 36; ++p) ot[p * 128 + otid] = u[p];
+        __syncthreads();
+        const int C = fwd ? d.Co : d.Ci, c0 = fwd ? co0 : ci0;
+        const long gbase = (long)((fwd ? ci0 : co0) / 4 + q) * 18;
+        const int nrow = min(P4_T, C - c0);
+#pragma unroll
+        for (int k = 0; k < 9; ++k) {
+            const int f = tid + k * 128, pq = f >> 6, hh = (f >> 5) & 1, row = f & 31;
+            if (row < nrow) {
+                const float* o0 = ot + f4_pos(pq, 0) * 128 + hh * 64 + row * 2;
+                const float* o1 = ot + f4_pos(pq, 1) * 128 + hh * 64 + row * 2;
+                *reinterpret_cast<f32x4*>(dst + (((gbase + pq) * 2 + hh) * C + c0 + row) * 4) =
+                    f32x4{o0[0], o0[1], o1[0], o1[1]};
+            }
+        }
+        __syncthreads();
+    }
+}
+
+struct WinoPackDesc {
+    const float* w; float* uf; float* ud;
+    int Co, Ci, ci_pad, co_pad;
+    long block_start;
+};
+
+__device__ __forceinline__ void wino_g(const float g[9], float u[16]) {
+    float t[12];
+#pragma unroll
+    for (int c = 0; c < 3; ++c) {
+        const float g0 = g[c], g1 = g[3 + c], g2 = g[6 + c];
+        t[c] = g0; t[3 + c] = 0.5f * (g0 + g1 + g2); t[6 + c] = 0.5f * (g0 - g1 + g2); t[9 + c] = g2;
+    }
+#pragma unroll
+    for (int r = 0; r < 4; ++r) {
+        const float a0 = t[r * 3], a1 = t[r * 3 + 1], a2 = t[r * 3 + 2];
+        u[r * 4] = a0; u[r * 4 + 1] = 0.5f * (a0 + a1 + a2); u[r * 4 + 2] = 0.5f * (a0 - a1 + a2); u[r * 4 + 3] = a2;
+    }
+}
+
+constexpr int WP_T = 32, WP_THREADS = 256, WP_OT = 16 * 256;
+template <class Taps>
+__device__ __forceinline__ void wino_pack_tile(const WinoPackDesc& d, int co0, int ci0, float* ot, Taps&& taps) {
+    const int tid = threadIdx.x;
+    const int nci = min(WP_T, d.Ci - ci0);
+    float g[9], u[16];
+    const int lo3 = tid & 7, hi5 = tid >> 3;
+    for (int grp = 0; grp < 8; ++grp) {
+        const bool fwd = grp < 4;
+        const int q = grp & 3;
+        float* dst = fwd ? d.uf : d.ud;
+        if (dst == nullptr) continue;
+        const int co = fwd ? hi5 : 8 * q + lo3, ci = fwd ? 8 * q + lo3 : hi5;
+        const bool live = fwd ? (ci0 + 8 * q < d.ci_pad) : (co0 + 8 * q < d.co_pad);
+        if (!live) continue;
+        {
+            const bool in = co0 + co < d.Co && ci < nci;
+            const float* wp = taps(co, ci);
+#pragma unroll
+            for (int t = 0; t < 9; ++t) g[t] = in ? wp[fwd ? t : 8 - t] : 0.f;
+        }
+        wino_g(g, u);
+#pragma unroll
+        for (int p = 0; p < 16; ++p) ot[p * 256 + tid] = u[p];
+        __syncthreads();
+        const int C = fwd ? d.Co : d.Ci, c0 = fwd ? co0 : ci0;
+        const long gbase = (long)((fwd ? ci0 : co0) / 8 + q) * 16;
+        const int nrun = min(WP_T, C - c0) * 8;
+#pragma unroll
+        for (int k = 0; k < 4; ++k) {
+            const int f = tid + k * 256, p = f >> 6, x4 = (f & 63) * 4;
+            if (x4 < nrun)
+                *reinterpret_cast<f32x4*>(dst + ((gbase + p) * C + c0) * 8 + x4) =
+                    *reinterpret_cast<const f32x4*>(ot + p * 256 + x4);
+        }
+        __syncthreads();
+    }
+}
+
+template <class Desc>
+__device__ __forceinline__ int pack_desc_of(const Desc* __restrict__ descs, int n, long blk) {
+    int lo = 0, hi = n - 1;
+    while (lo < hi) {
+        const int mid = (lo + hi + 1) >> 1;
+        if (descs[mid].block_start <= blk) lo = mid; else hi = mid - 1;
+    }
+    return lo;
+}
+
+}
diff --git a/aide_amd/engine.py b/aide_amd/engine.py
--- a/aide_amd/engine.py
+++ b/aide_amd/engine.py
@@ -1,4 +1,5 @@
 import ctypes
+import weakref
 
 import torch
 
@@ -8,6 +9,70 @@
 
 PARAM_EPOCH = [0]
 STATS_EPOCH = [0]
+
+
+PACK_LINKS = {}
+PACK_LINKS_EPOCH = [0]
+
+
+class PackLink(object):
+    __slots__ = ('param', 'shared', 'packs')
+
+    def __init__(self, param, shared):
+        self.param, self.shared, self.packs = param, shared, {}
+
+
+def pack_link(p):
+    link = PACK_LINKS.get(id(p))
+    return link if (link is not None and link.param() is p) else None
+
+
+def _forget_link(pid):
+    link = PACK_LINKS.get(pid)
+    if link is not None and link.param() is None:
+        del PACK_LINKS[pid]
+        PACK_LINKS_EPOCH[0] += 1
+
+
+def _register_packs(plan):
+    shared = plan._shared
+    convs = [st for st in plan.steps if st['kind'] == 'conv']
+    shared['wslots'] = [st['conv']._parameters for st in convs]
+    changed = False
+    for st in convs:
+        w = st['conv'].weight
+        for i, direction in enumerate('fd'):
+            mode = st['wino_' + direction]
+            t = st[_pack_slot(mode, direction)] if mode in (2, 4) else None
+            if t is None:
+                continue
+            link = pack_link(w)
+            if link is None or link.shared is not shared:
+                pid = id(w)
+                link = PACK_LINKS[pid] = PackLink(weakref.ref(w, lambda _, pid=pid: _forget_link(pid)), shared)
+                changed = True
+            slot = link.packs.setdefault(mode, [None, None])
+            if slot[i] is not t:
+                slot[i] = t
+                changed = True
+    if changed:
+        PACK_LINKS_EPOCH[0] += 1
+
+
+def _unregister_packs(shared):
+    dead = [pid for pid, link in PACK_LINKS.items() if link.shared is shared]
+    for pid in dead:
+        del PACK_LINKS[pid]
+    if dead:
+        PACK_LINKS_EPOCH[0] += 1
+
+
+def packs_refreshed(shared, pack_ids, stream):
+    key = (PARAM_EPOCH[0],) + tuple((w.data_ptr(), w._version) for w in [d['weight'] for d in shared['wslots']])
+    fresh = shared['fresh']
+    for i in pack_ids:
+        fresh[i] = key
+    shared['streams'] = (stream, None)
 
 
 class GTensor(object):
@@ -88,6 +153,7 @@
         fuse_head_bwd=True,
         lazy_head=True,
         fuse_pool_fwd=True,
+        fused_adam_pack=False,
     )
 
     def __init__(self, on_change=None):
@@ -329,12 +395,15 @@
         self._convs = self._conv_wslots = None
         self._gate_conv = None
         self._tape_f = self._tape_b = None
+        self._tape_gated = False
         self._coef_key, self._coef_tensors, self._coef_ok, self._coef_next, self._coef_bns = None, None, False, None, []
         self._fp = None
         self._fp_slots = self._fp_bns = None
         self.overlap = True
         self.trace = None
         self.serial = 0
+        if shared is not None and training and groups == 1 and cfg.fused_adam_pack:
+            _register_packs(self)
         self.key = None
 
     def _plan_lazy_bn(self):
@@ -666,10 +735,11 @@
         dyn = list(inputs) + [out]
         key = (torch.cuda.current_stream().cuda_stream, self._fp, tuple((tuple(t.shape), t.stride()) for t in dyn))
         tp = self._tape_f
-        if tp is not None and tp.key == key:
+        if tp is not None and tp.key == key and (gate is None or self._tape_gated):
             tp.replay(dyn, skip_tags=(() if gate is not None else ('gate',)) + (('aide_bn_eval_fold',) if self._coef_ok else ()))
             return out
         tp = Tape(key)
+        self._tape_gated = gate is not None
         with tp:
             self._forward_impl(inputs, out, gate, tp)
         self._tape_f = tp.finish(dyn)
@@ -1239,6 +1309,10 @@
 
     def _config_changed(self):
         self.plans = {}
+        self._drop_packs()
+
+    def _drop_packs(self):
+        _unregister_packs(self._shared_packs)
         self._shared_packs = dict(buf={}, fresh={}, streams=None)
 
     def grad_arena(self, device, fresh=False):
@@ -1260,7 +1334,7 @@
         if value != self._precision:
             self._precision = value
             self.plans = {}
-            self._shared_packs = dict(buf={}, fresh={}, streams=None)
+            self._drop_packs()
 
     def _refresh_params(self):
         slots = self._pslots
@@ -1289,7 +1363,7 @@
                 off += (params[i].numel() + 3) // 4 * 4
             self.flat_numel = off
             self.plans = {}
-            self._shared_packs = dict(buf={}, fresh={}, streams=None)
+            self._drop_packs()
             self._arena = self._views = None
 
     @staticmethod
diff --git a/aide_amd/ops.py b/aide_amd/ops.py
--- a/aide_amd/ops.py
+++ b/aide_amd/ops.py
@@ -664,6 +664,22 @@
     check(getattr(lib, 'aide_' + fam.pack_multi)(ptr(tab[0]), tab[1], tab[2], stream_ptr()), fam.pack_multi)
 
 
+def adam_pack_table(fam, entries, device):
+    rec, start = b'', 0
+    for p, m, v, vmax, uf, ud in entries:
+        co, ci = p.shape[0], p.shape[1]
+        rows = [t.shape[0] if (fam.pack_padded and t is not None) else 0 for t in (uf, ud)]
+        rec += struct.pack('<QQQQQQiiiiq', *([t.data_ptr() if t is not None else 0 for t in (p, m, v, vmax, uf, ud)] +
+                                             [co, ci, rows[0], rows[1], start]))
+        start += fam.pack_blocks(co, ci, uf, ud)
+    return torch.frombuffer(bytearray(rec), dtype=torch.uint8).to(device), len(entries), start
+
+
+def adam_pack(fam, tab, gtab, lr, beta1, beta2, eps, weight_decay, amsgrad, step):
+    check(lib.aide_adam_pack_multi(ptr(tab[0]), ptr(gtab), tab[1], tab[2], fam.mode, float(lr), float(beta1), float(beta2),
+                                   float(eps), float(weight_decay), int(bool(amsgrad)), step, stream_ptr()), 'adam_pack_multi')
+
+
 def _pack_one(fam, w, need_dgrad):
     _req(w)
     co, ci = w.shape[0], w.shape[1]
diff --git a/aide_amd/optim.py b/aide_amd/optim.py
--- a/aide_amd/optim.py
+++ b/aide_amd/optim.py
@@ -4,6 +4,7 @@
 
 from . import engine
 from ._lib import lib, check
+from . import ops
 from .ops import stream_ptr, ptr
 
 
@@ -44,12 +45,19 @@
                                           int(bool(group['amsgrad'])), step, stream_ptr()), 'adam')
 
     def _static_table(self, slot, plist):
-        st = [self.state[p] for p in plist]
-        key = tuple((p.data_ptr(), p.numel(), s['exp_avg'].data_ptr(), s['exp_avg_sq'].data_ptr(),
-                     s['max_exp_avg_sq'].data_ptr() if 'max_exp_avg_sq' in s else 0) for p, s in zip(plist, st))
+        key = self._table_key(plist)
         tab = self._tables.get(slot)
         if tab is not None and tab['key'] == key:
             return tab
+        tab = self._tables[slot] = self._make_table(plist, key)
+        return tab
+
+    def _table_key(self, plist):
+        st = [self.state[p] for p in plist]
+        return tuple((p.data_ptr(), p.numel(), s['exp_avg'].data_ptr(), s['exp_avg_sq'].data_ptr(),
+                      s['max_exp_avg_sq'].data_ptr() if 'max_exp_avg_sq' in s else 0) for p, s in zip(plist, st))
+
+    def _make_table(self, plist, key):
         dev = plist[0].device
         sizes = [p.numel() for p in plist]
         starts, acc = [], 0
@@ -62,8 +70,45 @@
         tab = dict(key=key, total_blocks=acc,
                    p=table([k[0] for k in key]), m=table([k[2] for k in key]), v=table([k[3] for k in key]),
                    vmax=table([k[4] for k in key]), sizes=table(sizes), starts=table(starts))
-        self._tables[slot] = tab
         return tab
+
+    def _split(self, fast, group):
+        epoch = engine.PACK_LINKS_EPOCH[0]
+        cached = fast.get('split')
+        if cached is not None and cached[0] == epoch:
+            return cached[1]
+        params, gkey = group['params'], fast['gkey']
+        dev = params[0].device
+        by_mode, plain = {}, []
+        for i, p in enumerate(params):
+            link = engine.pack_link(p) if engine.PACK_LINKS else None
+            if link is None or p.dim() != 4 or tuple(p.shape[2:]) != (3, 3):
+                plain.append(i)
+            else:
+                mode = 4 if 4 in link.packs else 2
+                by_mode.setdefault(mode, []).append((i, link))
+        split = None
+        if by_mode:
+            def gtable(idx):
+                return torch.tensor([gkey[i] for i in idx], dtype=torch.int64).to(dev)
+            fused, marks = [], {}
+            for mode, items in sorted(by_mode.items()):
+                entries = []
+                for i, link in items:
+                    p, st = params[i], self.state[params[i]]
+                    uf, ud = link.packs[mode]
+                    entries.append((p, st['exp_avg'], st['exp_avg_sq'], st.get('max_exp_avg_sq') if fast['amsgrad'] else None,
+                                    uf, ud))
+                    ids = marks.setdefault(id(link.shared), (link.shared, []))[1]
+                    ids += [id(t) for t in (uf, ud) if t is not None]
+                fam = ops.FAMILIES[mode]
+                fused.append((fam, ops.adam_pack_table(fam, entries, dev), gtable([i for i, _ in items])))
+            plist = [params[i] for i in plain]
+            split = dict(fused=fused, marks=list(marks.values()), n_plain=len(plist),
+                         tab=self._make_table(plist, self._table_key(plist)) if plist else None,
+                         gtab=gtable(plain) if plist else None)
+        fast['split'] = (epoch, split)
+        return split
 
     def _grad_table(self, slot, grads):
         gkey = tuple(g.data_ptr() for g in grads)
@@ -89,7 +134,7 @@
         if closure is not None:
             with torch.enable_grad():
                 loss = closure()
-        keep = []
+        keep, refreshed = [], []
         for gi, group in enumerate(self.param_groups):
             fast = self._fast.get(gi)
             if fast is not None:
@@ -102,7 +147,17 @@
                     step = fast['step'] = fast['step'] + 1
                     for st in fast['states']:
                         st['step'] = step
-                    self._launch(fast['tab'], fast['gtab'], fast['n'], group, step)
+                    split = self._split(fast, group)
+                    if split is None:
+                        self._launch(fast['tab'], fast['gtab'], fast['n'], group, step)
+                    else:
+                        b1, b2 = group['betas']
+                        for fam, tab, gtab in split['fused']:
+                            ops.adam_pack(fam, tab, gtab, group['lr'], b1, b2, group['eps'], group['weight_decay'],
+                                          group['amsgrad'], step)
+                        if split['tab'] is not None:
+                            self._launch(split['tab'], split['gtab'], split['n_plain'], group, step)
+                        refreshed += split['marks']
                     keep.append(fast['gtab'])
                     continue
                 self._fast.pop(gi, None)
@@ -147,4 +202,8 @@
                                                for s in states])
         self._keep = keep
         engine.PARAM_EPOCH[0] += 1
+        if refreshed:
+            cur = torch.cuda.current_stream()
+            for shared, ids in refreshed:
+                engine.packs_refreshed(shared, ids, cur)
         return loss
diff --git a/include/aide_hip.h b/include/aide_hip.h
--- a/include/aide_hip.h
+++ b/include/aide_hip.h
@@ -364,6 +364,9 @@
                             int ntensors, int64_t total_blocks, float lr, float beta1, float beta2,
                             float eps, float weight_decay, int amsgrad, int64_t step,
                             aide_stream_t stream);
+int aide_adam_pack_multi(const void* descs, const float* const* grads, int n, int64_t total_blocks, int family,
+                         float lr, float beta1, float beta2, float eps, float weight_decay, int amsgrad,
+                         int64_t step, aide_stream_t stream);
 
 #ifdef __cplusplus
 }
```

After: 645.1 images/sec (median of 2 runs). No clear change (-0.1%).
